# bbaaii/HFA-GP

Measured on AMD Instinct MI355X. Metric: rendered 512^2 frames/sec (96 depth samples), whole job, higher is better.
Workload: dtype f32 (conv GEMM products as f16x3: split 16-bit operands, fp32 accumulate); 1 GPU; ffhq512_128: synthesis fwd, 512^2 out, 128^2 rays x (48+48) samples, random-init weights (BASELINE config 2); parallelism=frame-parallel x1, conv_precision=f16x3

## Files before the change

hfa-gp_amd/_lib.py:

```python
from __future__ import annotations

import ctypes as C
import os
import threading

_HERE = os.path.dirname(os.path.abspath(__file__))
LIB_PATH = os.environ.get("HFAGP_LIB_PATH") or os.path.join(_HERE, "libhfagp_hip.so")
ABI_VERSION = 15

c_float_p = C.c_void_p


class RaymarchArgs(C.Structure):
    _fields_ = [
        ("planes", C.c_void_p), ("cam2world", C.c_void_p), ("intrinsics", C.c_void_p),
        ("u_strat", C.c_void_p), ("u_imp", C.c_void_p),
        ("dec_w0", C.c_void_p), ("dec_b0", C.c_void_p), ("dec_w1", C.c_void_p), ("dec_b1", C.c_void_p),
        ("feat", C.c_void_p), ("depth", C.c_void_p), ("wsum", C.c_void_p), ("tminmax", C.c_void_p),
        ("B", C.c_int32), ("H", C.c_int32), ("W", C.c_int32), ("res", C.c_int32),
        ("Sc", C.c_int32), ("Sf", C.c_int32), ("plane_axes", C.c_int32), ("white_back", C.c_int32),
        ("ray_start", C.c_double), ("ray_end", C.c_double),
        ("box_warp", C.c_float), ("decoder_lr_mul", C.c_float),
        ("planes_absmax", C.c_void_p), ("state", C.c_void_p),
    ]
# ... 90 lines not shown
class TorgbFinishArgs(C.Structure):
    _fields_ = [(n, C.c_void_p) for n in ("part", "bias", "rgb_in", "rgb_out", "y_pre")] + \
        [(n, C.c_int32) for n in ("nparts", "B", "H", "W", "Cout")] + [("clamp", C.c_float)]


class PointwiseBwdArgs(C.Structure):
    _fields_ = [(n, C.c_void_p) for n in (
        "dxs_conv", "s_conv", "dxs_rgb", "s_rgb", "g_rgb_small", "w_rgb_small", "s_small", "g_direct", "x",
        "dcoef_p", "bias_p", "noise_p", "g_out", "partial", "sums")] + \
        [(n, C.c_int32) for n in ("B", "H", "W", "C", "Co", "nchunks", "has_producer", "act_p", "param_grads")] + \
        [(n, C.c_float) for n in ("noise_strength_p", "alpha", "gain", "clamp")] + \
        [(n, C.c_void_p) for n in ("y_rgb_small", "g_nchw3_a", "g_nchw3_b")] + [("clamp_rgb_small", C.c_float)] + \
        [("noise_strength_dev", C.c_void_p)]


class StyleBwdArgs(C.Structure):
    _fields_ = [(n, C.c_void_p) for n in ("ds", "dd", "styles", "dcoef", "wsq", "affine_w", "dstot", "dw")] + \
        [(n, C.c_int32) for n in ("B", "Cin", "Cout", "w_dim", "dw_stride", "accumulate")] + \
        [("style_gain", C.c_float)]


class WgradArgs(C.Structure):
    _fields_ = [(n, C.c_void_p) for n in ("x", "styles", "g", "weight", "dd", "dcoef", "dweight", "workspace")] + \
        [(n, C.c_int32) for n in ("B", "H", "W", "Cin", "Cout", "mode", "ksplit", "precision", "accumulate", "dd_stride")]


class AffineGradItem(C.Structure):
    _fields_ = [(n, C.c_void_p) for n in ("dstot", "w", "dA", "db")] + [(n, C.c_int32) for n in ("B", "Cin", "w_dim", "w_stride")]


class ReducePartialsItem(C.Structure):
    _fields_ = [("partial", C.c_void_p), ("sums", C.c_void_p)] + [(n, C.c_int32) for n in ("B", "nchunks", "n")]


class BiasNoiseGradItem(C.Structure):
    _fields_ = [(n, C.c_void_p) for n in ("sums", "dbias", "dnoise")] + [(n, C.c_int32) for n in ("B", "C")]


class WeightPrepItem(C.Structure):
    _fields_ = [(n, C.c_void_p) for n in ("weight", "image", "image_t", "wsq")] + \
        [(n, C.c_int32) for n in ("Cout", "Cin", "taps", "precision", "precision_t")] + [("w_absmax", C.c_void_p)]


class StyleBwdItem(C.Structure):
    _fields_ = [(n, C.c_void_p) for n in ("ds", "dd", "styles", "dcoef", "wsq", "affine_w", "dstot", "dw")] + \
        [(n, C.c_int32) for n in ("B", "Cin", "Cout", "w_dim", "dw_stride", "ds_stride", "dd_stride")] + \
        [("style_gain", C.c_float)]


class RaymarchBwdArgs(C.Structure):
    _fields_ = [("fwd", RaymarchArgs), ("g_feat", C.c_void_p), ("d_planes", C.c_void_p), ("rec", C.c_void_p),
                ("d_dec_w0", C.c_void_p), ("d_dec_b0", C.c_void_p), ("d_dec_w1", C.c_void_p), ("d_dec_b1", C.c_void_p),
                ("df_scratch", C.c_void_p), ("rows_scratch", C.c_void_p), ("rows_scratch_bytes", C.c_uint64)]


class RaymarchGeomGrads(C.Structure):
    _fields_ = [("g_depth", C.c_void_p), ("g_wsum", C.c_void_p), ("depth_range", C.c_void_p)]


SYMBOLS = {
    "hfagp_abi_version": (C.c_int, []),
    "hfagp_last_error": (C.c_char_p, []),
    "hfagp_raymarch_fwd": (C.c_int, [C.POINTER(RaymarchArgs), C.c_void_p]),
    "hfagp_raymarch_normals": (C.c_int, [C.POINTER(RaymarchArgs), C.c_void_p, C.c_void_p]),
    "hfagp_raymarch_normals_bwd": (C.c_int, [C.POINTER(RaymarchArgs)] + [C.c_void_p] * 7),
    "hfagp_raymarch_normals_bwd_camera": (C.c_int, [C.POINTER(RaymarchArgs), C.c_void_p, C.c_void_p, C.c_int] + [C.c_void_p] * 3),
    "hfagp_planes_query": (C.c_int, [C.POINTER(PlanesQueryArgs), C.c_void_p]),
    "hfagp_planes_query_bwd": (C.c_int, [C.POINTER(PlanesQueryBwdArgs), C.c_void_p]),
    "hfagp_planes_query_normals": (C.c_int, [C.POINTER(PlanesQueryArgs), C.c_void_p, C.c_void_p, C.c_void_p]),
    "hfagp_planes_query_normals_bwd": (C.c_int, [C.POINTER(PlanesQueryBwdArgs), C.c_void_p, C.c_void_p, C.c_void_p]),
    "hfagp_marching_cubes_workspace_bytes": (C.c_size_t, [C.c_int32] * 3),
    "hfagp_marching_cubes_count": (C.c_int, [C.POINTER(MarchingCubesArgs), C.c_void_p]),
    "hfagp_marching_cubes_emit": (C.c_int, [C.POINTER(MarchingCubesArgs), C.c_void_p]),
    "hfagp_depth_clamp": (C.c_int, [C.c_void_p, C.c_void_p, C.c_int64, C.c_void_p]),
    "hfagp_style_fwd": (C.c_int, [C.POINTER(StyleArgs), C.c_void_p]),
    "hfagp_fc_fwd": (C.c_int, [C.c_void_p] * 4 + [C.c_int32] * 3 + [C.c_float, C.c_int32, C.c_float, C.c_float, C.c_void_p]),
    "hfagp_weight_prep": (C.c_int, [C.c_void_p, C.c_void_p, C.c_void_p, C.c_int32, C.c_int32, C.c_int32, C.c_void_p]),
    "hfagp_qr_gram_fwd": (C.c_int, [C.c_void_p, C.c_void_p, C.c_void_p, C.c_void_p, C.c_int32, C.c_void_p]),
    "hfagp_qr_refine_fwd": (C.c_int, [C.c_void_p, C.c_void_p, C.c_void_p, C.c_void_p, C.c_int32, C.c_void_p]),
    "hfagp_tall_gram_workspace_bytes": (C.c_size_t, [C.c_int32, C.c_int32]),
    "hfagp_tall_gram": (C.c_int, [C.c_void_p, C.c_int64, C.c_int64, C.c_void_p, C.c_int64, C.c_int64, C.c_void_p, C.c_void_p,
                                  C.c_int32, C.c_int32, C.c_float, C.c_void_p]),
    "hfagp_style_batch_fwd": (C.c_int, [C.POINTER(StyleArgs), C.c_int32, C.c_void_p]),
    "hfagp_weight_prep_split": (C.c_int, [C.c_void_p, C.c_void_p, C.c_int32, C.c_int32, C.c_int32, C.c_int32, C.c_void_p]),
    "hfagp_weight_prep_prec": (C.c_int, [C.c_void_p, C.c_void_p, C.c_int32, C.c_int32, C.c_int32, C.c_int32, C.c_void_p]),
    "hfagp_weight_prep_scaled": (C.c_int, [C.c_void_p, C.c_void_p, C.c_void_p, C.c_int32, C.c_int32, C.c_int32, C.c_int32, C.c_void_p]),
    "hfagp_modconv_workspace_bytes": (C.c_size_t, [C.POINTER(ModconvArgs)]),
    "hfagp_modconv_fwd": (C.c_int, [C.POINTER(ModconvArgs), C.c_void_p]),
    "hfagp_upfir_epilogue_fwd": (C.c_int, [C.POINTER(UpfirEpilogueArgs), C.c_void_p]),
    "hfagp_upconv_fir_scratch_bytes": (C.c_size_t, [C.POINTER(ModconvArgs)]),
    "hfagp_upconv_fir_fwd": (C.c_int, [C.POINTER(ModconvArgs), C.c_void_p, C.c_void_p]),
    "hfagp_skip_upsample_add": (C.c_int, [C.POINTER(SkipArgs), C.c_void_p]),
    "hfagp_torgb_skip_fwd": (C.c_int, [C.POINTER(TorgbSkipArgs), C.c_void_p]),
    "hfagp_blur_down_fwd": (C.c_int, [C.c_void_p, C.c_void_p, C.c_int32, C.c_int32, C.c_int32, C.c_int32, C.c_void_p]),
    "hfagp_blur_down_bwd": (C.c_int, [C.c_void_p, C.c_void_p, C.c_int32, C.c_int32, C.c_int32, C.c_int32, C.c_void_p]),
    "hfagp_torgb_fwd": (C.c_int, [C.POINTER(TorgbArgs), C.c_void_p]),
    "hfagp_torgb_finish_fwd": (C.c_int, [C.POINTER(TorgbFinishArgs), C.c_void_p]),
    "hfagp_modconv_rgb_parts": (C.c_int32, [C.POINTER(ModconvArgs)]),
    "hfagp_pointwise_bwd": (C.c_int, [C.POINTER(PointwiseBwdArgs), C.c_void_p]),
    "hfagp_upfir_bwd": (C.c_int, [C.c_void_p, C.c_void_p] + [C.c_int32] * 4 + [C.c_void_p]),
    "hfagp_upsample2d_bwd": (C.c_int, [C.c_void_p, C.c_void_p, C.c_int64, C.c_int32, C.c_int32, C.c_int32, C.c_void_p]),
    "hfagp_planes_to_nhwc": (C.c_int, [C.c_void_p, C.c_void_p] + [C.c_int32] * 4 + [C.c_void_p]),
    "hfagp_style_bwd": (C.c_int, [C.POINTER(StyleBwdArgs), C.c_void_p]),
    "hfagp_style_batch_bwd": (C.c_int, [C.POINTER(StyleBwdItem), C.c_int32, C.c_void_p]),
    "hfagp_raymarch_bwd": (C.c_int, [C.POINTER(RaymarchBwdArgs), C.c_void_p]),
    "hfagp_raymarch_bwd_geom": (C.c_int, [C.POINTER(RaymarchBwdArgs), C.POINTER(RaymarchGeomGrads), C.c_void_p]),
    "hfagp_raymarch_bwd_rows_bytes": (C.c_size_t, [C.POINTER(RaymarchArgs)]),
    "hfagp_raymarch_bwd_camera": (C.c_int, [C.POINTER(RaymarchBwdArgs), C.c_void_p, C.c_void_p, C.c_void_p, C.c_void_p]),
    "hfagp_adam_step": (C.c_int, [C.c_void_p, C.c_void_p, C.c_int32, C.c_int32, C.c_double, C.c_double, C.c_double, C.c_double, C.c_void_p]),
    "hfagp_adam_chunk": (C.c_int32, []),
    "hfagp_weight_prep_batch": (C.c_int, [C.POINTER(WeightPrepItem), C.c_int32, C.c_void_p]),
    "hfagp_wgrad_ksplit": (C.c_int32, [C.POINTER(WgradArgs)]),
    "hfagp_wgrad_workspace_bytes": (C.c_size_t, [C.POINTER(WgradArgs)]),
    "hfagp_conv_wgrad": (C.c_int, [C.POINTER(WgradArgs), C.c_void_p]),
    "hfagp_affine_grad": (C.c_int, [C.c_void_p] * 4 + [C.c_int32] * 4 + [C.c_void_p]),
    "hfagp_affine_grad_batch": (C.c_int, [C.POINTER(AffineGradItem), C.c_int32, C.c_void_p]),
    "hfagp_bias_noise_grads": (C.c_int, [C.POINTER(BiasNoiseGradItem), C.c_int32, C.c_void_p]),
    "hfagp_reduce_partials_batch": (C.c_int, [C.POINTER(ReducePartialsItem), C.c_int32, C.c_void_p]),
    "hfagp_channel_sum": (C.c_int, [C.c_void_p] * 3 + [C.c_int64, C.c_int32, C.c_int32, C.c_int32, C.c_void_p]),
    "hfagp_pool_mse_workspace_bytes": (C.c_size_t, []),
    "hfagp_pool_mse_fwd": (C.c_int, [C.c_void_p] * 5 + [C.c_int32] * 4 + [C.c_void_p]),
    "hfagp_pool_mse_bwd": (C.c_int, [C.c_void_p] * 4 + [C.c_int32] * 4 + [C.c_void_p]),
    "hfagp_upfirdn2d_fwd": (C.c_int, [C.c_void_p, C.c_void_p, C.c_void_p] + [C.c_int32] * 12 + [C.c_float, C.c_void_p]),
    "hfagp_upfirdn2d_bwd": (C.c_int, [C.c_void_p, C.c_void_p, C.c_void_p] + [C.c_int32] * 12 + [C.c_float, C.c_void_p]),
    "hfagp_bias_act_bwd": (C.c_int, [C.c_void_p, C.c_void_p, C.c_void_p, C.c_int64, C.c_int32, C.c_float, C.c_float,
                                     C.c_float, C.c_void_p]),
    "hfagp_bias_act_fwd": (C.c_int, [C.c_void_p, C.c_void_p, C.c_void_p, C.c_int64, C.c_int32, C.c_int64,
                                     C.c_int32, C.c_float, C.c_float, C.c_float, C.c_void_p]),
    "hfagp_allreduce_f32": (C.c_int, [C.c_void_p, C.c_size_t, C.c_void_p, C.c_int32, C.c_void_p]),
    "hfagp_nchw_to_nhwc": (C.c_int, [C.c_void_p, C.c_void_p] + [C.c_int32] * 4 + [C.c_void_p]),
    "hfagp_nhwc_to_nchw": (C.c_int, [C.c_void_p, C.c_void_p] + [C.c_int32] * 4 + [C.c_void_p]),
}

_lock = threading.Lock()
_lib = None


def lib() -> C.CDLL:
    global _lib
    if _lib is not None:
        return _lib
    with _lock:
        if _lib is not None:
            return _lib
        if not os.path.exists(LIB_PATH):
            raise RuntimeError(
                f"hfa_gp_amd: HIP library not found at {LIB_PATH}. There is no CPU fallback; build it with "
                f"`bash {os.path.join(_HERE, 'csrc', 'build.sh')}` (hipcc --offload-arch=gfx950).")
        try:
            import torch
            handle = C.CDLL(LIB_PATH)
        except OSError as e:
            raise RuntimeError(f"hfa_gp_amd: cannot load {LIB_PATH}: {e}") from e
        for name, (res, args) in SYMBOLS.items():
            try:
                fn = getattr(handle, name)
            except AttributeError as e:
                raise RuntimeError(f"hfa_gp_amd: {LIB_PATH} does not export {name}") from e
            fn.restype = res
            fn.argtypes = args
        ver = handle.hfagp_abi_version()
        if ver != ABI_VERSION:
            raise RuntimeError(f"hfa_gp_amd: ABI version mismatch: library {ver}, binding {ABI_VERSION}")
        _lib = handle
    return _lib

# ... 6 lines not shown
```

hfa-gp_amd/csrc/elementwise.hip:

```cpp
#include "common.h"

namespace hfagp {

static thread_local char g_err[512] = "";
void set_error(const char* fmt, ...) {
    va_list ap;
    va_start(ap, fmt);
    vsnprintf(g_err, sizeof(g_err), fmt, ap);
    va_end(ap);
}

__global__ void __launch_bounds__(256) style_kernel(const float* __restrict__ w, const float* __restrict__ A,
                                                    const float* __restrict__ ab, float* __restrict__ styles,
                                                    int B, int w_dim, int w_stride, int Cin, float wgain, float sgain) {
    const int wave = (blockIdx.x * blockDim.x + threadIdx.x) >> 6;
    const int lane = threadIdx.x & 63;
    if (wave >= B * Cin) return;
    const int b = wave / Cin, i = wave % Cin;
    const float* wr = w + (size_t)b * w_stride;
    const float* ar = A + (size_t)i * w_dim;
    float acc = 0.f;
    for (int k = lane * 4; k < w_dim; k += 256) {
        const float4 x = *reinterpret_cast<const float4*>(wr + k);
        const float4 y = *reinterpret_cast<const float4*>(ar + k);
        acc += x.x * y.x + x.y * y.y + x.z * y.z + x.w * y.w;
    }
    for (int o = 32; o > 0; o >>= 1) acc += __shfl_xor(acc, o);
    if (lane == 0) styles[wave] = (acc * wgain + ab[i]) * sgain;
}

__global__ void __launch_bounds__(256) demod_kernel(const float* __restrict__ styles, const float* __restrict__ wsq,
                                                    float* __restrict__ dcoef, int B, int Cin, int Cout, float eps) {
    const int wave = (blockIdx.x * blockDim.x + threadIdx.x) >> 6;
    const int lane = threadIdx.x & 63;
    if (wave >= B * Cout) return;
    const int b = wave / Cout, o = wave % Cout;
    const float* s = styles + (size_t)b * Cin;
    const float* q = wsq + (size_t)o * Cin;
    float acc = 0.f;
    for (int k = lane; k < Cin; k += 64) acc += s[k] * s[k] * q[k];
    for (int m = 32; m > 0; m >>= 1) acc += __shfl_xor(acc, m);
    if (lane == 0) dcoef[wave] = rsqrtf(acc + eps);
}

constexpr int kStyleBatch = 32;
struct StyleBatch { HfagpStyleArgs it[kStyleBatch]; };

__global__ void __launch_bounds__(256) style_batch_kernel(const StyleBatch t) {
    const HfagpStyleArgs& a = t.it[blockIdx.y];
    const int wave = (blockIdx.x * blockDim.x + threadIdx.x) >> 6;
    const int lane = threadIdx.x & 63;
    if (wave >= a.B * a.Cin) return;
    const int b = wave / a.Cin, i = wave % a.Cin;
    const float* wr = a.w + (size_t)b * a.w_stride;
    const float* ar = a.affine_w + (size_t)i * a.w_dim;
    float acc = 0.f;
    for (int k = lane * 4; k < a.w_dim; k += 256) {
        const float4 x = *reinterpret_cast<const float4*>(wr + k);
        const float4 y = *reinterpret_cast<const float4*>(ar + k);
        acc += x.x * y.x + x.y * y.y + x.z * y.z + x.w * y.w;
    }
    for (int o = 32; o > 0; o >>= 1) acc += __shfl_xor(acc, o);
    if (lane == 0) a.styles[wave] = (acc * rsqrtf((float)a.w_dim) + a.affine_b[i]) * a.style_gain;
}

__global__ void __launch_bounds__(256) demod_batch_kernel(const StyleBatch t) {
    const HfagpStyleArgs& a = t.it[blockIdx.y];
    if (!a.dcoef) return;
    const int wave = (blockIdx.x * blockDim.x + threadIdx.x) >> 6;
    const int lane = threadIdx.x & 63;
    if (wave >= a.B * a.Cout) return;
    const int b = wave / a.Cout, o = wave % a.Cout;
    const float* s = a.styles + (size_t)b * a.Cin;
    const float* q = a.wsq + (size_t)o * a.Cin;
    float acc = 0.f;
    for (int k = lane; k < a.Cin; k += 64) acc += s[k] * s[k] * q[k];
    for (int m = 32; m > 0; m >>= 1) acc += __shfl_xor(acc, m);
    if (lane == 0) a.dcoef[wave] = rsqrtf(acc + a.eps);
}

__global__ void __launch_bounds__(256) fc_kernel(const float* __restrict__ x, const float* __restrict__ W,
                                                 const float* __restrict__ bias, float* __restrict__ y, int B, int In,
                                                 int Out, float wgain, float bgain, int act, float alpha, float gain) {
    const int wave = (blockIdx.x * blockDim.x + threadIdx.x) >> 6, lane = threadIdx.x & 63;
    if (wave >= B * Out) return;
    const int b = wave / Out, o = wave % Out;
    float acc = 0.f;
    for (int k = lane; k < In; k += 64) acc += x[(size_t)b * In + k] * W[(size_t)o * In + k];
    for (int m = 32; m > 0; m >>= 1) acc += __shfl_xor(acc, m);
    if (lane == 0) y[wave] = lrelu_gain_clamp(acc * wgain + (bias ? bias[o] * bgain : 0.f), act, alpha, gain, -1.f);
}

__global__ void __launch_bounds__(256) weight_prep_kernel(const float* __restrict__ w, float* __restrict__ wt,
                                                          float* __restrict__ wsq, int Cout, int Cin, int taps) {
    const int idx = blockIdx.x * blockDim.x + threadIdx.x;
    if (idx >= Cout * Cin) return;
    const int co = idx / Cin, ci = idx % Cin;
    const float* src = w + (size_t)idx * taps;
    float sq = 0.f;
    for (int t = 0; t < taps; ++t) {
        const float v = src[t];
        sq += v * v;
        wt[(((size_t)t * (Cin >> 2) + (ci >> 2)) * Cout + co) * 4 + (ci & 3)] = v;
    }
    if (wsq) wsq[idx] = sq;
}

#ifndef HFAGP_FIR_STRIP
#define HFAGP_FIR_STRIP 8
#endif
constexpr int kStrip = HFAGP_FIR_STRIP;

typedef _Float16 h2_t __attribute__((ext_vector_type(2)));
typedef float f2_t __attribute__((ext_vector_type(2)));
template <bool H16>
__device__ __forceinline__ float4 load4(const void* base, size_t idx4) {
    if constexpr (H16) {
        const uint2 u = reinterpret_cast<const uint2*>(base)[idx4];
        const h2_t a = __builtin_bit_cast(h2_t, u.x), b = __builtin_bit_cast(h2_t, u.y);
        return make_float4((float)a[0], (float)a[1], (float)b[0], (float)b[1]);
    } else {
        return reinterpret_cast<const float4*>(base)[idx4];
    }
}
template <bool H16>
__device__ __forceinline__ void store4(void* base, size_t idx4, float4 v) {
    if constexpr (H16) {
        const f2_t lo = {v.x, v.y}, hi = {v.z, v.w};
        reinterpret_cast<uint2*>(base)[idx4] = make_uint2(__builtin_bit_cast(unsigned, __builtin_convertvector(lo, h2_t)),
                                                          __builtin_bit_cast(unsigned, __builtin_convertvector(hi, h2_t)));
    } else {
        reinterpret_cast<float4*>(base)[idx4] = v;
    }
}

template <bool H16>
__global__ void __launch_bounds__(256) upfir_epilogue_kernel(HfagpUpfirEpilogueArgs a) {
    const int C4 = a.C >> 2;
    const int Wo = 2 * a.W, Ho = 2 * a.H, Wi = 2 * a.W + 1, Hi = 2 * a.H + 1;
    const int Wp = a.W;
    const int strips = (Ho + kStrip - 1) / kStrip;
    const long long total = (long long)a.B * strips * Wp * C4;
    const long long tid = (long long)blockIdx.x * blockDim.x + threadIdx.x;
    if (tid >= total) return;
    const int c4 = (int)(tid % C4);
    const int X = 2 * (int)((tid / C4) % Wp);
    const int st = (int)((tid / ((long long)C4 * Wp)) % strips);
    const int b = (int)(tid / ((long long)C4 * Wp * strips));
    const int Y0 = st * kStrip;
    const size_t src0 = (size_t)b * Hi * Wi * C4 + c4;
    const float f0 = 0.25f, f1 = 0.75f;

    int xo[5]; float xm[5];
#pragma unroll
// ... 313 lines not shown
    for (int p = 0; p < fh; ++p) {
        const int uy = oy * down + p - py0;
        if (uy < 0 || uy % up != 0) continue;
        const int iy = uy / up;
        if (iy >= H) continue;
        for (int q = 0; q < fw; ++q) {
            const int ux = ox * down + q - px0;
            if (ux < 0 || ux % up != 0) continue;
            const int ix = ux / up;
            if (ix >= W) continue;
            acc += (noflip ? f[p * fw + q] : f[(fh - 1 - p) * fw + (fw - 1 - q)]) * src[(size_t)iy * W + ix];
        }
    }
    y[tid] = acc * gain;
}

__global__ void __launch_bounds__(256) bias_act_kernel(const float* __restrict__ x, const float* __restrict__ b,
                                                       float* __restrict__ y, long long n, int C, long long inner,
                                                       int act, float alpha, float gain, float clamp) {
    const long long stride = (long long)gridDim.x * blockDim.x;
    for (long long i = (long long)blockIdx.x * blockDim.x + threadIdx.x; i < n; i += stride) {
        float v = x[i];
        if (b) v += b[(i / inner) % C];
        y[i] = lrelu_gain_clamp(v, act, alpha, gain, clamp);
    }
}

__global__ void __launch_bounds__(256) bias_act_bwd_kernel(const float* __restrict__ dy, const float* __restrict__ y,
                                                           float* __restrict__ dx, long long n, int act, float alpha,
                                                           float gain, float clamp) {
    const long long stride = (long long)gridDim.x * blockDim.x;
    for (long long i = (long long)blockIdx.x * blockDim.x + threadIdx.x; i < n; i += stride) {
        const float yv = y[i];
        float g = dy[i] * gain;
        if (act == HFAGP_ACT_LRELU && !(yv > 0.f)) g *= alpha;
        if (clamp >= 0.f && !(fabsf(yv) < clamp)) g = 0.f;
        dx[i] = g;
    }
}

__global__ void __launch_bounds__(256) transpose_kernel(const float* __restrict__ x, float* __restrict__ y,
                                                        int rows, int cols) {
    __shared__ float tile[32][33];
    const size_t base = (size_t)blockIdx.z * rows * cols;
    const int c0 = blockIdx.x * 32, r0 = blockIdx.y * 32;
    const int tx = threadIdx.x & 31, ty = threadIdx.x >> 5;
    for (int k = ty; k < 32; k += 8) {
        const int r = r0 + k, c = c0 + tx;
        if (r < rows && c < cols) tile[k][tx] = x[base + (size_t)r * cols + c];
    }
    __syncthreads();
    for (int k = ty; k < 32; k += 8) {
        const int c = c0 + k, r = r0 + tx;
        if (r < rows && c < cols) y[base + (size_t)c * rows + r] = tile[tx][k];
    }
}

}

using namespace hfagp;

extern "C" {

int hfagp_abi_version(void) { return HFAGP_ABI_VERSION; }
const char* hfagp_last_error(void) { return g_err; }

int hfagp_style_fwd(const HfagpStyleArgs* a, void* stream) {
    HFAGP_REQUIRE(a && a->w && a->affine_w && a->affine_b && a->styles, HFAGP_EBADARG, "style_fwd: null pointer");
    HFAGP_REQUIRE(a->B > 0 && a->Cin > 0 && a->w_dim > 0 && a->w_dim % 4 == 0 && a->w_stride % 4 == 0,
                  HFAGP_EBADARG, "style_fwd: bad dims B=%d Cin=%d w_dim=%d", a->B, a->Cin, a->w_dim);
    hipStream_t s = (hipStream_t)stream;
    const float wgain = 1.0f / sqrtf((float)a->w_dim);
    int waves = a->B * a->Cin;
    style_kernel<<<(waves + 3) / 4, 256, 0, s>>>(a->w, a->affine_w, a->affine_b, a->styles, a->B, a->w_dim,
                                                 a->w_stride, a->Cin, wgain, a->style_gain);
    if (a->dcoef) {
        HFAGP_REQUIRE(a->wsq && a->Cout > 0, HFAGP_EBADARG, "style_fwd: dcoef requested without wsq");
        waves = a->B * a->Cout;
        demod_kernel<<<(waves + 3) / 4, 256, 0, s>>>(a->styles, a->wsq, a->dcoef, a->B, a->Cin, a->Cout, a->eps);
    }
    return check_launch("style_fwd");
}

int hfagp_style_batch_fwd(const HfagpStyleArgs* items, int32_t n, void* stream) {
    HFAGP_REQUIRE(items && n >= 1 && n <= kStyleBatch, HFAGP_EBADARG, "style_batch_fwd: 1..%d items, got %d", kStyleBatch, n);
    StyleBatch t;
    int max_s = 0, max_d = 0;
    for (int i = 0; i < n; ++i) {
        const HfagpStyleArgs& a = items[i];
        HFAGP_REQUIRE(a.w && a.affine_w && a.affine_b && a.styles, HFAGP_EBADARG, "style_batch_fwd: null pointer in item %d", i);
        HFAGP_REQUIRE(a.B > 0 && a.Cin > 0 && a.w_dim > 0 && a.w_dim % 4 == 0 && a.w_stride % 4 == 0, HFAGP_EBADARG,
                      "style_batch_fwd: bad dims in item %d: B=%d Cin=%d w_dim=%d", i, a.B, a.Cin, a.w_dim);
        HFAGP_REQUIRE(!a.dcoef || (a.wsq && a.Cout > 0), HFAGP_EBADARG, "style_batch_fwd: item %d: dcoef without wsq", i);
        t.it[i] = a;
        max_s = a.B * a.Cin > max_s ? a.B * a.Cin : max_s;
        if (a.dcoef) max_d = a.B * a.Cout > max_d ? a.B * a.Cout : max_d;
    }
    hipStream_t s = (hipStream_t)stream;
    style_batch_kernel<<<dim3((max_s + 3) / 4, n), 256, 0, s>>>(t);
    if (max_d) demod_batch_kernel<<<dim3((max_d + 3) / 4, n), 256, 0, s>>>(t);
    return check_launch("style_batch_fwd");
}

int hfagp_fc_fwd(const float* x, const float* weight, const float* bias, float* y, int32_t B, int32_t In, int32_t Out,
                 float lr_mul, int32_t act, float alpha, float gain, void* stream) {
    HFAGP_REQUIRE(x && weight && y, HFAGP_EBADARG, "fc_fwd: null pointer");
    HFAGP_REQUIRE(B > 0 && In > 0 && Out > 0, HFAGP_EBADARG, "fc_fwd: bad dims");
    HFAGP_REQUIRE(act == HFAGP_ACT_LINEAR || act == HFAGP_ACT_LRELU, HFAGP_EUNSUPPORTED, "fc_fwd: act %d", act);
    const int waves = B * Out;
    fc_kernel<<<(waves + 3) / 4, 256, 0, (hipStream_t)stream>>>(x, weight, bias, y, B, In, Out,
                                                                lr_mul / sqrtf((float)In), lr_mul, act, alpha, gain);
    return check_launch("fc_fwd");
}

int hfagp_weight_prep(const float* weight, float* wt, float* wsq, int32_t Cout, int32_t Cin, int32_t taps,
                      void* stream) {
    HFAGP_REQUIRE(weight && wt, HFAGP_EBADARG, "weight_prep: null pointer");
    HFAGP_REQUIRE(Cin % 4 == 0 && Cout > 0 && (taps == 1 || taps == 9), HFAGP_EUNSUPPORTED,
                  "weight_prep: Cin=%d must be a multiple of 4, taps=%d must be 1 or 9", Cin, taps);
    const int n = Cout * Cin;
    weight_prep_kernel<<<(n + 255) / 256, 256, 0, (hipStream_t)stream>>>(weight, wt, wsq, Cout, Cin, taps);
    return check_launch("weight_prep");
}

int hfagp_upfir_epilogue_fwd(const HfagpUpfirEpilogueArgs* a, void* stream) {
    HFAGP_REQUIRE(a && a->yt && a->y, HFAGP_EBADARG, "upfir_epilogue: null pointer");
    HFAGP_REQUIRE(a->C % 4 == 0 && a->B > 0 && a->H > 0 && a->W > 0, HFAGP_EUNSUPPORTED,
                  "upfir_epilogue: C=%d must be a multiple of 4", a->C);
    const int strips = (2 * a->H + kStrip - 1) / kStrip;
    const long long total = (long long)a->B * strips * a->W * (a->C / 4);
    if (a->io_f16) upfir_epilogue_kernel<true><<<(unsigned)((total + 255) / 256), 256, 0, (hipStream_t)stream>>>(*a);
    else upfir_epilogue_kernel<false><<<(unsigned)((total + 255) / 256), 256, 0, (hipStream_t)stream>>>(*a);
    return check_launch("upfir_epilogue");
}

int hfagp_skip_upsample_add(const HfagpSkipArgs* a, void* stream) {
    HFAGP_REQUIRE(a && a->y && a->img_out, HFAGP_EBADARG, "skip_upsample_add: null pointer");
    HFAGP_REQUIRE(a->C % 4 == 0 && (!a->plane_major || (a->C % 3 == 0 && (a->C / 3) % 4 == 0)), HFAGP_EUNSUPPORTED,
                  "skip_upsample_add: unsupported channel count %d", a->C);
    const int Ho = a->img_in ? 2 * a->H : a->H, Wo = a->img_in ? 2 * a->W : a->W;
    const long long total = (long long)a->B * Ho * Wo * (a->C / 4);
    skip_kernel<<<(unsigned)((total + 255) / 256), 256, 0, (hipStream_t)stream>>>(*a);
    return check_launch("skip_upsample_add");
}

int hfagp_torgb_fwd(const HfagpTorgbArgs* a, void* stream) {
    HFAGP_REQUIRE(a && a->x && a->weight && a->styles && a->bias && a->rgb_out, HFAGP_EBADARG, "torgb: null pointer");
    HFAGP_REQUIRE(a->Cout >= 1 && a->Cout <= kTorgbMaxOut && a->Cin % 4 == 0 && a->H % 2 == 0 && a->W % 2 == 0,
                  HFAGP_EUNSUPPORTED, "torgb: Cout=%d (max %d), Cin=%d", a->Cout, kTorgbMaxOut, a->Cin);
    const int HW = a->H * a->W;
    hipStream_t s = (hipStream_t)stream;
    const dim3 rgrid((HW + 32 * kTorgbIter - 1) / (32 * kTorgbIter), a->B);
    switch (a->Cin) {
        case 64:  if (a->Cout <= 3) torgb_reg_kernel<2, 3><<<rgrid, 256, 0, s>>>(*a); else torgb_reg_kernel<2, 4><<<rgrid, 256, 0, s>>>(*a); break;
        case 128: if (a->Cout <= 3) torgb_reg_kernel<4, 3><<<rgrid, 256, 0, s>>>(*a); else torgb_reg_kernel<4, 4><<<rgrid, 256, 0, s>>>(*a); break;
        case 256: if (a->Cout <= 3) torgb_reg_kernel<8, 3><<<rgrid, 256, 0, s>>>(*a); else torgb_reg_kernel<8, 4><<<rgrid, 256, 0, s>>>(*a); break;
        default: {
            dim3 grid((HW + 31) / 32, a->B);
            const size_t lds = (size_t)a->Cout * a->Cin * sizeof(float);
            torgb_kernel<<<grid, 256, lds, s>>>(*a);
        }
    }
    return check_launch("torgb");
}

int hfagp_torgb_finish_fwd(const HfagpTorgbFinishArgs* a, void* stream) {
    HFAGP_REQUIRE(a && a->part && a->bias && a->rgb_out, HFAGP_EBADARG, "torgb_finish: null pointer");
    HFAGP_REQUIRE(a->Cout >= 1 && a->Cout <= 3 && a->nparts >= 1 && a->H % 2 == 0 && a->W % 2 == 0, HFAGP_EUNSUPPORTED,
                  "torgb_finish: Cout=%d (max 3), nparts=%d", a->Cout, a->nparts);
    const long long total = (long long)a->B * a->H * a->W;
    torgb_finish_kernel<<<(unsigned)((total + 255) / 256), 256, 0, (hipStream_t)stream>>>(*a);
    return check_launch("torgb_finish");
}

int hfagp_blur_down_fwd(const float* x, float* y, int32_t B, int32_t H, int32_t W, int32_t C, void* stream) {
    HFAGP_REQUIRE(x && y, HFAGP_EBADARG, "blur_down: null pointer");
    HFAGP_REQUIRE(B > 0 && H > 0 && W > 0 && H % 2 == 0 && W % 2 == 0 && C % 4 == 0, HFAGP_EUNSUPPORTED,
                  "blur_down: H=%d, W=%d must be even and C=%d a multiple of 4", H, W, C);
    const long long total = (long long)B * (H / 2) * (W / 2) * (C / 4);
    blur_down_kernel<<<(unsigned)((total + 255) / 256), 256, 0, (hipStream_t)stream>>>(x, y, B, H, W, C / 4);
    return check_launch("blur_down_fwd");
}

int hfagp_blur_down_bwd(const float* gy, float* gx, int32_t B, int32_t H, int32_t W, int32_t C, void* stream) {
// ... 72 lines not shown
```

hfa-gp_amd/csrc/modconv.hip:

```cpp
#include "modconv_plan.h"

namespace hfagp {

typedef float f32x16 __attribute__((ext_vector_type(16)));

constexpr int CK = 8;
constexpr int AS = 12;
constexpr int LPW = 32;

template <int WM, int WN, int TM, int TN>
__global__ void __launch_bounds__(256) modconv_kernel(const ConvParams p) {
    constexpr int BM = WM * TM * 32, BN = WN * TN * 32, PH = BM / PW;
    extern __shared__ __attribute__((aligned(16))) float lds[];
    float* As = lds;
    float* Bs = lds + ((PH + 2) * LPW) * AS;

    const Phase& ph = p.phase[blockIdx.y];
    unsigned id = blockIdx.x;
    const int tn_blk = __builtin_amdgcn_readfirstlane(id % p.tiles_n); id /= p.tiles_n;
    const int tw = __builtin_amdgcn_readfirstlane(id % p.tiles_w);     id /= p.tiles_w;
    const int th = __builtin_amdgcn_readfirstlane(id % p.tiles_h);     id /= p.tiles_h;
    const int b = __builtin_amdgcn_readfirstlane(id % p.B);            id /= p.B;
    const int ks = __builtin_amdgcn_readfirstlane(id);
    const int m0 = th * PH, n0 = tw * PW, co0 = tn_blk * BN;
    if (m0 >= ph.mh || n0 >= ph.mw) return;

    const int tid = threadIdx.x, lane = tid & 63, wave = tid >> 6;
    const int wm = wave / WN, wn = wave % WN;
    const int h = lane >> 5, l31 = lane & 31;

    const int c_begin = __builtin_amdgcn_readfirstlane((int)(((long long)p.nchunks * ks) / p.ksplit));
    const int c_end = __builtin_amdgcn_readfirstlane((int)(((long long)p.nchunks * (ks + 1)) / p.ksplit));

    const int npatch = p.ph * p.pw;
    constexpr int A_PER_T = ((PH + 2) * (PW + 2) * 2 + 255) / 256;
    constexpr int B_PER_T = (MAXTAPS * 2 * BN + 255) / 256;
    float4 ra[A_PER_T], rs[A_PER_T], rb[B_PER_T];
    const float* xb = p.x + ph.in_off + (long long)b * p.x_batch_stride;
    const float* sb = p.styles ? p.styles + (size_t)b * p.Cin : nullptr;
    const int nB = ph.ntaps * 2 * BN;
    const int cq = p.Cin >> 2;

    long long aoff[A_PER_T], boff[B_PER_T];
    int lds_a[A_PER_T];
#pragma unroll
    for (int k = 0; k < A_PER_T; ++k) {
        const int idx = tid + k * 256;
        aoff[k] = -1;
        lds_a[k] = 0;
        if (idx < npatch * 2) {
            const int pix = idx >> 1, q = idx & 1;
            lds_a[k] = ((pix / p.pw) * LPW + pix % p.pw) * AS + 4 * q;
            const int iy = m0 + p.dymin + pix / p.pw, ix = n0 + p.dxmin + pix % p.pw;
            if (iy >= 0 && iy < p.in_h && ix >= 0 && ix < p.in_w) aoff[k] = ((long long)iy * p.in_w + ix) * p.Cin + 4 * q;
        }
    }
#pragma unroll
    for (int k = 0; k < B_PER_T; ++k) {
        const int idx = tid + k * 256;
        boff[k] = -1;
        if (idx < nB) {
            const int co = idx % BN, q = (idx / BN) & 1, t = idx / (2 * BN);
            if (co0 + co < p.Cout) boff[k] = ((long long)ph.widx[t] * cq + q) * p.Cout + co0 + co;
        }
    }

    auto load_regs = [&](int chunk) {
        const int c0 = chunk * CK;
#pragma unroll
        for (int k = 0; k < A_PER_T; ++k) {
            float4 v = make_float4(0.f, 0.f, 0.f, 0.f), sv = make_float4(1.f, 1.f, 1.f, 1.f);
            if (aoff[k] >= 0) {
                v = *reinterpret_cast<const float4*>(xb + aoff[k] + c0);
                if (sb) sv = *reinterpret_cast<const float4*>(sb + c0 + 4 * ((tid + k * 256) & 1));
            }
            ra[k] = v; rs[k] = sv;
        }
#pragma unroll
        for (int k = 0; k < B_PER_T; ++k) {
            float4 v = make_float4(0.f, 0.f, 0.f, 0.f);
            if (boff[k] >= 0) v = reinterpret_cast<const float4*>(p.wt)[boff[k] + (long long)(c0 >> 2) * p.Cout];
            rb[k] = v;
        }
// ... 90 lines not shown
                const int m = m0 + (pidx >> 4), n = n0 + (pidx & 15);
                if (m >= ph.mh || n >= ph.mw) continue;
                const int oy = ph.sy * m + ph.oy0, ox = ph.sx * n + ph.ox0;
                float v = acc[tm][tn][r];
                if (p.fused) {
                    v = v * d + bs + nz[r] * p.noise_strength;
                    v = lrelu_gain_clamp(v, p.act, p.alpha, p.gain, p.clamp);
                }
                vmax = fmaxf(vmax, fabsf(v));
                out[(((size_t)b * p.Ho + oy) * p.Wo + ox) * p.Cout + co] = v;
            }
        }
    }
    if (p.fused && p.y_absmax) publish_absmax(p.y_absmax, vmax, blockIdx.x * 4 + (threadIdx.x >> 6));
}

__global__ void __launch_bounds__(256) splitk_epilogue_kernel(const float* __restrict__ ws, float* __restrict__ y,
                                                              const float* __restrict__ dcoef,
                                                              const float* __restrict__ noise,
                                                              const float* __restrict__ bias, long long slab,
                                                              int ksplit, int HoWo, int Cout, int fused, int act,
                                                              float noise_strength, float alpha, float gain,
                                                              float clamp, float* __restrict__ y_absmax) {
    const long long i4 = (long long)blockIdx.x * blockDim.x + threadIdx.x;
    if (i4 * 4 >= slab) return;
    float4 s = reinterpret_cast<const float4*>(ws)[i4];
    int k = 1;
    for (; k + 8 <= ksplit; k += 8) {
        float4 v[8];
#pragma unroll
        for (int q = 0; q < 8; ++q) v[q] = reinterpret_cast<const float4*>(ws + (size_t)(k + q) * slab)[i4];
#pragma unroll
        for (int q = 0; q < 8; ++q) { s.x += v[q].x; s.y += v[q].y; s.z += v[q].z; s.w += v[q].w; }
    }
    for (; k < ksplit; ++k) {
        const float4 v = reinterpret_cast<const float4*>(ws + (size_t)k * slab)[i4];
        s.x += v.x; s.y += v.y; s.z += v.z; s.w += v.w;
    }
    if (fused) {
        const long long e = i4 * 4;
        const int co = (int)(e % Cout);
        const long long pix = e / Cout;
        const int b = (int)(pix / HoWo);
        float4 d = make_float4(1.f, 1.f, 1.f, 1.f), bs = make_float4(0.f, 0.f, 0.f, 0.f);
        if (dcoef) d = *reinterpret_cast<const float4*>(dcoef + (size_t)b * Cout + co);
        if (bias) bs = *reinterpret_cast<const float4*>(bias + co);
        const float nz = noise ? noise[pix % HoWo] * noise_strength : 0.f;
        s.x = lrelu_gain_clamp(s.x * d.x + bs.x + nz, act, alpha, gain, clamp);
        s.y = lrelu_gain_clamp(s.y * d.y + bs.y + nz, act, alpha, gain, clamp);
        s.z = lrelu_gain_clamp(s.z * d.z + bs.z + nz, act, alpha, gain, clamp);
        s.w = lrelu_gain_clamp(s.w * d.w + bs.w + nz, act, alpha, gain, clamp);
    }
    reinterpret_cast<float4*>(y)[i4] = s;
    if (fused && y_absmax)
        publish_absmax(y_absmax, fmaxf(fmaxf(fabsf(s.x), fabsf(s.y)), fmaxf(fabsf(s.z), fabsf(s.w))), blockIdx.x * 4 + (threadIdx.x >> 6));
}

}

using namespace hfagp;

extern "C" {

static int resolve_modconv(const HfagpModconvArgs* a, Plan& pl) {
    const int ck = a && a->precision != HFAGP_PREC_F32 ? 16 : CK;
    int rc = validate(a, ck);
    if (rc == HFAGP_OK) rc = make_plan(a, pl, ck);
    if (rc != HFAGP_OK) return rc;
    pl.small = smallconv_takes(a);
    if (pl.small) {
        pl.p.ksplit = smallconv_ksplit(a);
        pl.ws_bytes = pl.p.ksplit > 1 ? (size_t)pl.p.ksplit * pl.p.slab * sizeof(float) : 0;
    }
    return HFAGP_OK;
}

size_t hfagp_modconv_workspace_bytes(const HfagpModconvArgs* a) {
    Plan pl;
    return resolve_modconv(a, pl) == HFAGP_OK ? pl.ws_bytes : 0;
}

int32_t hfagp_modconv_rgb_parts(const HfagpModconvArgs* a) { return a ? ((a->Cout + 127) / 128) * 2 : 0; }

int hfagp_modconv_fwd(const HfagpModconvArgs* a, void* stream) {
    Plan pl;
    int rc = resolve_modconv(a, pl);
    if (rc != HFAGP_OK) return rc;
    ConvParams& p = pl.p;
    HFAGP_REQUIRE((a->rgb_w == nullptr) == (a->rgb_part == nullptr), HFAGP_EBADARG, "modconv: rgb_w and rgb_part go together");
    if (pl.small) {
        rc = launch_smallconv(a, pl, (hipStream_t)stream);
        if (rc != HFAGP_OK || p.ksplit == 1) return rc;
        const long long n4 = p.slab / 4;
        splitk_epilogue_kernel<<<(unsigned)((n4 + 255) / 256), 256, 0, (hipStream_t)stream>>>(
            a->workspace, a->y, a->dcoef, a->noise, a->bias, p.slab, p.ksplit, p.Ho * p.Wo, a->Cout, 1, a->act,
            a->noise_strength, a->alpha, a->gain, a->clamp, a->y_absmax);
        return check_launch("modconv_fwd/splitk (small-image kernel)");
    }
    HFAGP_REQUIRE(!a->rgb_part || (a->precision != HFAGP_PREC_F32 && p.ksplit * p.nslab == 1 && p.fused && a->Cout % 128 == 0 &&
                                   (a->mode == HFAGP_CONV3X3 || a->mode == HFAGP_CONV1X1)),
                  HFAGP_EUNSUPPORTED, "modconv: the fused toRGB needs a 16-bit precision, mode 0 / 2, Cout %% 128 == 0 and no "
                                      "split-K (workspace_bytes() == 0); got precision %d mode %d Cout %d ksplit %d",
                  a->precision, a->mode, a->Cout, p.ksplit);
    HFAGP_REQUIRE(a->y || (a->rgb_part && !a->y_absmax), HFAGP_EBADARG,
                  "modconv: y may only be NULL with the fused toRGB (rgb_w / rgb_part) and without y_absmax");
    hipStream_t s = (hipStream_t)stream;
    const int nslabs = p.ksplit * p.nslab;
    if (nslabs > 1) {
        HFAGP_REQUIRE(a->workspace, HFAGP_EBADARG, "modconv: split-K (%d slabs) needs a workspace of %zu bytes", nslabs,
                      pl.ws_bytes);
        p.out = a->workspace;
    } else {
        p.out = a->y;
    }
    HFAGP_REQUIRE(!(a->x_f16 || a->y_f16) || a->precision == HFAGP_PREC_F16, HFAGP_EUNSUPPORTED,
                  "modconv: fp16 storage (x_f16 / y_f16) goes with precision HFAGP_PREC_F16");
    if (a->precision != HFAGP_PREC_F32) {
        rc = launch_modconv_bf16(a, pl, s);
        if (rc != HFAGP_OK) return rc;
    } else {
        const size_t lds_bytes = ((size_t)(pl.bm / PW + 2) * LPW * AS + (size_t)MAXTAPS * 2 * pl.bn * 4) * sizeof(float);
        switch (pl.bn) {
            case 128: modconv_kernel<2, 2, 2, 2><<<pl.grid, 256, lds_bytes, s>>>(p); break;
            case 96:  modconv_kernel<4, 1, 1, 3><<<pl.grid, 256, lds_bytes, s>>>(p); break;
            case 64:  modconv_kernel<2, 2, 2, 1><<<pl.grid, 256, lds_bytes, s>>>(p); break;
            default:  modconv_kernel<4, 1, 1, 1><<<pl.grid, 256, lds_bytes, s>>>(p); break;
        }
        rc = check_launch("modconv_fwd");
        if (rc != HFAGP_OK) return rc;
    }
    if (nslabs > 1) {
        const int fused = a->mode != HFAGP_CONVT3X3_UP2 && a->mode != HFAGP_CONVS2_BWD;
        const long long n4 = p.slab / 4;
        splitk_epilogue_kernel<<<(unsigned)((n4 + 255) / 256), 256, 0, s>>>(
            a->workspace, a->y, a->dcoef, a->noise, a->bias, p.slab, nslabs, p.Ho * p.Wo, a->Cout, fused, a->act,
            a->noise_strength, a->alpha, a->gain, a->clamp, a->y_absmax);
        rc = check_launch("modconv_fwd/splitk");
    }
    return rc;
}

}
```

hfa-gp_amd/csrc/modconv_bf16.hip:

```cpp
#include <atomic>
#include <type_traits>
#include "conv16_common.h"

namespace hfagp {

template <int KD, int TM, int NTAPS, int IO = 0>
__global__ void __launch_bounds__(256, 2) modconv_bf16_kernel(const ConvParams p, const int phase0) {
    constexpr int NP = kind_parts_a(KD), NPB = kind_parts(KD);
    constexpr bool F16 = kind_f16(KD);
    constexpr bool XH = (IO & 1) != 0, YH = (IO & 2) != 0;
    constexpr int XB = XH ? 2 : 4;
    static_assert((IO & 3) == 0 || KD == 1, "fp16 storage goes with the single-pass fp16 arithmetic");
    constexpr bool ELEG = (IO & 4) != 0;
    static_assert(!ELEG || (KD == 4 && NTAPS == 9 && IO == 4), "the legacy epilogue is kept for one instantiation");
    constexpr int WN = 2, WM = 4 / WN, TN = 4 / WN, TMW = 4 / WM, BM = 128, PH = BM / PW;
    static_assert(TM == 2, "block tile is 128 positions");
    constexpr int LPWB = RowPitch<NP>::value;
    constexpr int APOS = (PH + 2) * LPWB;
    constexpr int A_PART = APOS * APITCH, A_BUF = NP * A_PART;
    extern __shared__ __attribute__((aligned(16))) char lds_raw[];
    char* As = lds_raw;
    float* Ss = reinterpret_cast<float*>(lds_raw + 2 * A_BUF);

    constexpr bool MERGED_S2 = NTAPS == 0;
// ... 342 lines not shown
            for (int rw = 0; rw < 2; ++rw) {
                const int m = m0 + 2 * (wm * TMW + tm) + rw;
                if (m >= ph.mh) continue;
                const int oy = ph.sy * m + ph.oy0;
                const size_t rowoff = (((size_t)b * p.Ho + oy) * p.Wo + ph.ox0) * p.Cout + co;
                float* rowp = out + rowoff;
                _Float16* rowh = reinterpret_cast<_Float16*>(p.out) + rowoff;
                const float* nrow = (p.fused && p.noise) ? p.noise + (size_t)oy * p.Wo + ph.ox0 : nullptr;
                float nz[8];
#pragma unroll
                for (int q = 0; q < 8; ++q) {
                    const int n = min(n0 + 8 * (q >> 2) + 4 * h + (q & 3), ph.mw - 1);
                    nz[q] = nrow ? nrow[ph.sx * n] * p.noise_strength : 0.f;
                }
#pragma unroll
                for (int q = 0; q < 8; ++q) {
                    const int n = n0 + 8 * (q >> 2) + 4 * h + (q & 3);
                    if (n >= ph.mw) continue;
                    float v = acc[tm][tn][8 * rw + q];
                    if (p.fused) v = lrelu_gain_clamp(v * d + bs + nz[q], p.act, p.alpha, p.gain, p.clamp);
                    else if constexpr (F16) v *= sback;
                    vmax = fmaxf(vmax, fabsf(v));
                    if (p.out) {
                        if constexpr (YH) rowh[n * cstep] = (_Float16)v;
                        else rowp[n * cstep] = v;
                    }
                    if constexpr (RGB) {
#pragma unroll
                        for (int r = 0; r < 3; ++r)
                            rgbp[((tm * 2 + rw) * 8 + q) * 3 + r] = fmaf(v, rw3[r], rgbp[((tm * 2 + rw) * 8 + q) * 3 + r]);
                    }
                }
            }
    }
    if (p.fused && p.y_absmax) publish_absmax(p.y_absmax, vmax, blockIdx.x * 4 + wave);
    }
    if constexpr (RGB) {
        if (do_rgb) {
            int n = TMW * 16 * 3;
#pragma unroll
            for (int m = 16; m >= 1; m >>= 1) {
                n >>= 1;
                const bool up = (l31 & m) != 0;
#pragma unroll
                for (int i = 0; i < TMW * 16 * 3 / 2; ++i) {
                    if (i < n) {
                        const float keep = up ? rgbp[i + n] : rgbp[i];
                        const float give = up ? rgbp[i] : rgbp[i + n];
                        rgbp[i] = keep + __shfl_xor(give, m);
                    }
                }
            }
            const int pos = l31;
            const int tm = pos >> 4, rw = (pos >> 3) & 1, q = pos & 7;
            const int m = m0 + 2 * (wm * TMW + tm) + rw, nn = n0 + 8 * (q >> 2) + 4 * h + (q & 3);
            if (m < ph.mh && nn < ph.mw) {
                const int part = tn_blk * WN + wn;
                float4* dst = reinterpret_cast<float4*>(p.rgb_part) +
                              (((size_t)part * p.B + b) * p.Ho + (ph.sy * m + ph.oy0)) * p.Wo + (ph.sx * nn + ph.ox0);
                *dst = make_float4(rgbp[0], rgbp[1], rgbp[2], 0.f);
            }
        }
    }
}

constexpr int UP4_OCC = 2;
template <int KD, int NW, int IO = 0>
__global__ void __launch_bounds__(NW * 64, (NW == 4 && KD != 3) ? UP4_OCC : 1) upconv_bf16_kernel(const ConvParams p) {
    constexpr int NP = kind_parts_a(KD), NPB = kind_parts(KD);
    constexpr bool F16 = kind_f16(KD);
    constexpr bool XH = (IO & 1) != 0, YH = (IO & 2) != 0;
    constexpr int XB = XH ? 2 : 4;
    static_assert(IO == 0 || KD == 1, "fp16 storage goes with the single-pass fp16 arithmetic");
    constexpr int NTH = NW * 64;
    constexpr int TM = 2, TN = 1, WN = NW / 2, BM = 128, BNU = WN * TN * 32, PH = BM / PW, RB = kind_nprod(KD) == 1 ? 6 : 3;
    constexpr int LPWB = RowPitch<NP>::value;
    constexpr int APOS = (PH + 2) * LPWB;
    constexpr int A_PART = APOS * APITCH, A_BUF = NP * A_PART;
    using namespace up_items;
    extern __shared__ __attribute__((aligned(16))) char lds_raw[];
    char* As = lds_raw;
    float* Ss = reinterpret_cast<float*>(lds_raw + 2 * A_BUF);

    unsigned id = p.xcd ? xcd_remap(blockIdx.x, gridDim.x) : blockIdx.x;
    const int tiles_nu = p.Cout / BNU;
    const int tn_blk = __builtin_amdgcn_readfirstlane(id % tiles_nu);  id /= tiles_nu;
    const int n_reg = p.up_tr * p.up_tw, n_tile = n_reg + p.up_nf;
    const int T = __builtin_amdgcn_readfirstlane(id % n_tile);         id /= n_tile;
    const int ks = __builtin_amdgcn_readfirstlane(id);
    const bool fringe = T >= n_reg;
    const int RP = p.up_rp, R_total = p.up_rows;
    const int r0 = fringe ? (T - n_reg) * 64 : (T / p.up_tw) * PH, n0 = fringe ? 0 : (T % p.up_tw) * PW;
    const int co0 = tn_blk * BNU;
    const int b_lo = min(max(r0 - 1, 0) / RP, p.B - 1);

    const int tid = threadIdx.x, lane = tid & 63, wave = tid >> 6;
    const int wm = wave / WN, wn = wave % WN;
    const int h = lane >> 5, l31 = lane & 31;
    const int c_begin = __builtin_amdgcn_readfirstlane((int)(((long long)p.nchunks * ks) / p.ksplit));
    const int c_end = __builtin_amdgcn_readfirstlane((int)(((long long)p.nchunks * (ks + 1)) / p.ksplit));

    const int npatch = p.ph * p.pw;
    constexpr int A_PER_T = ((PH + 2) * (PW + 2) * 4 + NTH - 1) / NTH;
    static_assert(A_PER_T == 2 || A_PER_T == 3, "staging schedule: two or three slots per thread");
    float4 ra[A_PER_T];
    const char* xb = reinterpret_cast<const char*>(p.x) + (long long)b_lo * p.x_batch_stride * XB;
    float* Gd = Ss + p.up_ns * p.Cin;
    {
        const long long s_lo = (long long)b_lo * p.Cin, s_n = (long long)p.B * p.Cin;
        for (int i = tid; i < p.up_ns * p.Cin; i += NTH) Ss[i] = (p.styles && s_lo + i < s_n) ? p.styles[s_lo + i] : 1.f;
        for (int sI = 0; sI < p.up_ns; ++sI) {
            float bk = 1.f, dn = 1.f;
            if constexpr (F16)
                dn = style_range_guard((p.styles && b_lo + sI < p.B) ? p.styles + (size_t)(b_lo + sI) * p.Cin : nullptr, p.Cin, lane, &bk,
                                       p.x_absmax, p.w_absmax);
            if (tid == 0) { Gd[sI] = dn; Gd[p.up_ns + sI] = bk; }
        }
    }
    __syncthreads();
    unsigned aoff[A_PER_T];
    int lds_a[A_PER_T], soff[A_PER_T];
    float amask[A_PER_T];
#pragma unroll
    for (int k = 0; k < A_PER_T; ++k) {
        const int idx = min(tid + k * NTH, npatch * 4 - 1);
        const int pix = idx >> 2, q = idx & 3;
        const int pi = pix / p.pw, pj = pix % p.pw;
        lds_a[k] = (pi * LPWB + pj) * APITCH + 8 * q;
        int r, n;
        if (!fringe) { r = r0 - 1 + pi; n = n0 - 1 + pj; }
        else { r = pj == 0 ? -1 : r0 + 8 * ((pj - 1) >> 1) + pi - 1; n = p.W - 1 + ((pj - 1) & 1); }
        const bool row_ok = r >= 0 && r < R_total;
        const int bb = row_ok ? r / RP : b_lo, m = r - bb * RP;
        const bool inside = row_ok && m < p.H && n >= 0 && n < p.W;
        const int sel = inside ? bb - b_lo : 0;
        aoff[k] = inside ? (unsigned)(((long long)sel * p.x_batch_stride + (long long)(m * p.W + n) * p.Cin + 4 * q) * XB) : 0u;
        amask[k] = inside ? Gd[sel] : 0.f;
        soff[k] = sel * p.Cin + 4 * q;
    }
    auto load_a = [&](int chunk) __attribute__((always_inline)) { a16_load<XH>(ra, xb, chunk, aoff); };
    auto store_a = [&](int chunk, auto buf_tag, auto k_tag) __attribute__((always_inline)) {
        constexpr int BUF = decltype(buf_tag)::value, k = decltype(k_tag)::value;
        a16_store<KD, XH>(As + BUF * A_BUF, A_PART, lds_a[k], amask[k], *reinterpret_cast<const float4*>(Ss + chunk * CKB + soff[k]), ra[k]);
    };

    const char* wb = reinterpret_cast<const char*>(p.wt);
    const int cq8 = p.Cin >> 3;
    const int part_stride = 9 * cq8 * p.Cout;
    unsigned bth[TN];
#pragma unroll
    for (int tn = 0; tn < TN; ++tn) bth[tn] = (unsigned)(h * p.Cout + co0 + (wn * TN + tn) * 32 + l31) * 16u;
    int apos[TM];
#pragma unroll
    for (int tm = 0; tm < TM; ++tm) {
        const int pidx = (wm * TM + tm) * 32 + l31;
        apos[tm] = ((pidx >> 4) * LPWB + (pidx & 15)) * APITCH + 16 * h;
    }

    f32x16 acc[4][TM][TN];
#pragma unroll
    for (int f = 0; f < 4; ++f)
#pragma unroll
        for (int tm = 0; tm < TM; ++tm)
#pragma unroll
            for (int tn = 0; tn < TN; ++tn)
#pragma unroll
                for (int r = 0; r < 16; ++r) acc[f][tm][tn][r] = 0.f;

    constexpr PartOrder PO = kind_order(KD);
    constexpr int NPROD = PO.nprod;
    u32x4 bq[RB][TN][NPB];
    u32x4 af[2][TM][NP];
    auto issue_b = [&](int c, auto i_tag, auto slot_tag) __attribute__((always_inline)) {
        constexpr int I = decltype(i_tag)::value, SL = decltype(slot_tag)::value;
        const int cc = min(c, c_end - 1);
#pragma unroll
        for (int q = 0; q < NPB; ++q) {
            const char* base = wb + (long long)(q * part_stride + (I_W[I] * cq8 + cc * 2) * p.Cout) * 16;
#pragma unroll
            for (int tn = 0; tn < TN; ++tn) bq[SL][tn][q] = *reinterpret_cast<const u32x4*>(base + bth[tn]);
        }
    };
    auto read_a = [&](auto u_tag, auto g_tag) __attribute__((always_inline)) {
        constexpr int UU = decltype(u_tag)::value, G = decltype(g_tag)::value;
#pragma unroll
        for (int tm = 0; tm < TM; ++tm)
#pragma unroll
            for (int q = 0; q < NP; ++q)
                af[G & 1][tm][q] = *reinterpret_cast<const u32x4*>(As + UU * A_BUF + q * A_PART + group_pos(G, LPWB) * APITCH + apos[tm]);
    };
    auto item = [&](int c, auto u_tag, auto i_tag) __attribute__((always_inline)) {
        constexpr int I = decltype(i_tag)::value, G = I_GRP[I], F = I_PHASE[I];
        constexpr int SL = (decltype(u_tag)::value * NITEM + I) % RB;
        if constexpr (I == G_FIRST[G] && G < 3) read_a(u_tag, std::integral_constant<int, G + 1>{});
        __builtin_amdgcn_sched_barrier(0);
#pragma unroll
        for (int pr = 0; pr < NPROD; ++pr)
#pragma unroll
            for (int tm = 0; tm < TM; ++tm)
// ... 366 lines not shown
    for (int tn = 0; tn < 4; ++tn) {
        const int co = co0 + wn * 64 + tn * 16 + i16;
        float rw3[3] = {0.f, 0.f, 0.f};
        if (do_rgb) {
#pragma unroll
            for (int r = 0; r < 3; ++r) rw3[r] = p.rgb_w[((size_t)b * 3 + r) * p.Cout + co];
        }
        float d = sback, bs = 0.f;
        if (p.fused) {
            if (p.dcoef) d = p.dcoef[(size_t)b * p.Cout + co] * sback;
            if (p.bias) bs = p.bias[co];
        }
#pragma unroll
        for (int tm = 0; tm < 4; ++tm) {
            const int m = m0 + 4 * wm + tm;
            if (m >= p.Ho) continue;
            float* rowp = out + ((size_t)b * p.Ho + m) * p.Wo * p.Cout + co;
            const float* nrow = (p.fused && p.noise) ? p.noise + (size_t)m * p.Wo : nullptr;
#pragma unroll
            for (int r = 0; r < 4; ++r) {
                const int n = n0 + 4 * g + r;
                const float nz = nrow ? nrow[min(n, p.Wo - 1)] * p.noise_strength : 0.f;
                if (n >= p.Wo) continue;
                float v = acc[tm][tn][r];
                if (p.fused) v = lrelu_gain_clamp(v * d + bs + nz, p.act, p.alpha, p.gain, p.clamp);
                else v *= sback;
                vmax = fmaxf(vmax, fabsf(v));
                if (p.out) rowp[n * p.Cout] = v;
#pragma unroll
                for (int c = 0; c < 3; ++c) rgbp[(tm * 4 + r) * 3 + c] = fmaf(v, rw3[c], rgbp[(tm * 4 + r) * 3 + c]);
            }
        }
    }
    if (p.fused && p.y_absmax) publish_absmax(p.y_absmax, vmax, blockIdx.x * 4 + wave);
    }
    if (do_rgb) {
        int n = 16 * 3;
#pragma unroll
        for (int mk = 8; mk >= 1; mk >>= 1) {
            n >>= 1;
            const bool up = (i16 & mk) != 0;
#pragma unroll
            for (int i = 0; i < 16 * 3 / 2; ++i) {
                if (i < n) {
                    const float keep = up ? rgbp[i + n] : rgbp[i];
                    const float give = up ? rgbp[i] : rgbp[i + n];
                    rgbp[i] = keep + __shfl_xor(give, mk);
                }
            }
        }
        const int m = m0 + 4 * wm + (i16 >> 2), nn = n0 + 4 * g + (i16 & 3);
        if (m < p.Ho && nn < p.Wo) {
            const int part = tn_blk * 2 + wn;
            float4* dst = reinterpret_cast<float4*>(p.rgb_part) + (((size_t)part * p.B + b) * p.Ho + m) * p.Wo + nn;
            *dst = make_float4(rgbp[0], rgbp[1], rgbp[2], 0.f);
        }
    }
}

namespace u16 {
constexpr int CK = 32;
constexpr int LP = PW + 1, NPOS = (8 + 1) * LP;
constexpr int OCT = 2560;
constexpr int A_PART = 4 * OCT, A_BUF = 2 * A_PART;
constexpr int A_PER_T = 5;
constexpr unsigned OOB = 0xfffff000u;
static_assert(NPOS * 16 <= OCT && OCT % 256 == 0 && NPOS * 8 <= A_PER_T * 256 && 2 * A_BUF <= 48 * 1024, "patch layout");
constexpr size_t lds_bytes(int cin, int ns) { return (size_t)2 * A_BUF + (size_t)ns * (cin + 1) * sizeof(float); }
}

template <int KD, int NW, int IO, int LOOP>
__global__ void __launch_bounds__(256, 2) upconv_bf16_kernel(const ConvParams p) {
    static_assert(KD == 4 && NW == 4 && IO == 0 && LOOP == 2, "the 32-channel loop is the 4-wave F16X3 up-conv");
    using namespace u16;
    typedef float f32x4v __attribute__((ext_vector_type(4)));
    using namespace up_items;
    constexpr int RB = 2;
    constexpr int ST = 0;
    constexpr int S_SLOT[NITEM] = {-1, -1, 0, 1, -1, 2, 3, -1, 4};
    extern __shared__ __attribute__((aligned(16))) char lds_raw[];
    char* As = lds_raw;
    float* Ss = reinterpret_cast<float*>(lds_raw + 2 * A_BUF);

    unsigned id = p.xcd ? xcd_remap(blockIdx.x, gridDim.x) : blockIdx.x;
    const int tiles_nu = p.Cout / 64;
    const int tn_blk = __builtin_amdgcn_readfirstlane(id % tiles_nu);  id /= tiles_nu;
    const int n_reg = p.up_tr * p.up_tw, n_tile = n_reg + p.up_nf;
    const int T = __builtin_amdgcn_readfirstlane(id % n_tile);         id /= n_tile;
    const int ks = __builtin_amdgcn_readfirstlane(id);
    const bool fringe = T >= n_reg;
    const int RP = p.up_rp, R_total = p.up_rows;
    const int r0 = fringe ? (T - n_reg) * 64 : (T / p.up_tw) * 8, n0 = fringe ? 0 : (T % p.up_tw) * PW;
    const int co0 = tn_blk * 64;
    const int b_lo = min(max(r0 - 1, 0) / RP, p.B - 1);

    const int tid = threadIdx.x, lane = tid & 63, wave = __builtin_amdgcn_readfirstlane(tid >> 6);
    const int wm = wave >> 1, wn = wave & 1;
    const int g = lane >> 4, i16 = lane & 15;
    const int nch = p.Cin / CK;
    const int c_begin = __builtin_amdgcn_readfirstlane((int)(((long long)nch * ks) / p.ksplit));
    const int c_end = __builtin_amdgcn_readfirstlane((int)(((long long)nch * (ks + 1)) / p.ksplit));

    float* Gb = Ss + p.up_ns * p.Cin;
    for (int sI = 0; sI < p.up_ns; ++sI) {
        const float* st = (p.styles && b_lo + sI < p.B) ? p.styles + (size_t)(b_lo + sI) * p.Cin : nullptr;
        float bk = 1.f;
        const float dn = style_range_guard(st, p.Cin, lane, &bk, p.x_absmax, p.w_absmax);
        for (int i = tid; i < p.Cin; i += 256) Ss[sI * p.Cin + i] = (st ? st[i] : 1.f) * dn;
        if (tid == 0) Gb[sI] = bk;
    }

    const int nsamp = min(p.up_ns, p.B - b_lo);
    const __amdgpu_buffer_rsrc_t rx = __builtin_amdgcn_make_buffer_rsrc(
        const_cast<float*>(p.x + (long long)b_lo * p.x_batch_stride), 0,
        (unsigned)(((long long)(nsamp - 1) * p.x_batch_stride + (long long)p.H * p.W * p.Cin) * 4), 0x00020000);
    const int qa = 2 * ((tid >> 4) & 3) + (tid & 1);
    static_assert(A_PART <= (1 << 14) && 14 + 3 * A_PER_T <= 32, "LDS address and sample indices share a register");
    unsigned aoff[A_PER_T];
    unsigned sels = (qa >> 1) * OCT + (8 * (tid >> 6) + ((tid >> 1) & 7)) * 16 + (qa & 1) * 8;
#pragma unroll
    for (int k = 0; k < A_PER_T; ++k) {
        const int pix = 8 * ((tid >> 6) + 4 * k) + ((tid >> 1) & 7);
        const int pi = pix / LP, pj = pix % LP;
        int r, n;
        if (!fringe) { r = r0 - 1 + pi; n = n0 - 1 + pj; }
        else { r = pj == 0 ? -1 : r0 + 8 * ((pj - 1) >> 1) + pi - 1; n = p.W - 1 + ((pj - 1) & 1); }
        const bool row_ok = r >= 0 && r < R_total;
        const int bb = row_ok ? r / RP : b_lo, m = r - bb * RP;
        const bool inside = pix < NPOS && row_ok && m < p.H && n >= 0 && n < p.W;
        const int sel = inside ? bb - b_lo : 0;
        aoff[k] = inside ? (unsigned)(((long long)sel * p.x_batch_stride + (long long)(m * p.W + n) * p.Cin + 4 * qa) * 4) : OOB;
        sels |= (unsigned)sel << (14 + 3 * k);
    }
    static_assert((8 * (3 + 4 * (A_PER_T - 1)) + 7) * 16 < OCT, "every slot lies inside its octet");
    float4 ra[2];
    auto load_a = [&](int chunk, auto part_tag) __attribute__((always_inline)) {
        constexpr int PT = decltype(part_tag)::value;
#pragma unroll
        for (int k = 0; k < (PT < 2 ? 2 : 1); ++k)
            ra[k] = __builtin_bit_cast(float4, __builtin_amdgcn_raw_buffer_load_b128(rx, aoff[PT * 2 + k], chunk * CK * 4, 0));
    };
    auto store_a = [&](int chunk, auto buf_tag, auto k_tag) __attribute__((always_inline)) {
        constexpr int BUF = decltype(buf_tag)::value, k = decltype(k_tag)::value;
        const int sel = (int)((sels >> (14 + 3 * k)) & 7u);
        const float4 sv = *reinterpret_cast<const float4*>(Ss + chunk * CK + sel * p.Cin + 4 * qa);
        const int lds_a = (int)(sels & 0x3fffu) + k * 32 * 16;
        const float4 x = ra[k % 2];
        uint2 parts[2];
        split4<KD>(make_float4(x.x * sv.x, x.y * sv.y, x.z * sv.z, x.w * sv.w), parts);
#pragma unroll
        for (int q = 0; q < 2; ++q) *reinterpret_cast<uint2*>(As + BUF * A_BUF + q * A_PART + lds_a) = parts[q];
    };

    const int cq8 = p.Cin >> 3;
    const __amdgpu_buffer_rsrc_t rw = __builtin_amdgcn_make_buffer_rsrc(
        const_cast<void*>(p.wt), 0, (unsigned)(2 * 9 * cq8 * p.Cout) * 16u, 0x00020000);
    const unsigned boff = (unsigned)(g * p.Cout + co0 + wn * 32 + i16) * 16u;
    const int part_bytes = 9 * cq8 * p.Cout * 16, tap_bytes = cq8 * p.Cout * 16, chunk_bytes = 4 * p.Cout * 16;
    const char* const afrag = As + g * OCT + (4 * wm * LP + i16) * 16;

    f32x4v acc[4][4][2];
#pragma unroll
    for (int f = 0; f < 4; ++f)
#pragma unroll
        for (int tm = 0; tm < 4; ++tm)
#pragma unroll
            for (int tn = 0; tn < 2; ++tn) acc[f][tm][tn] = f32x4v{0.f, 0.f, 0.f, 0.f};

    constexpr PartOrder PO = kind_order(KD);
    u32x4 bq[RB][2][2];
    u32x4 af[4][2];
    auto issue_b = [&](int c, int w, auto slot_tag) __attribute__((always_inline)) {
        constexpr int SL = decltype(slot_tag)::value;
#pragma unroll
        for (int q = 0; q < 2; ++q) {
            const int so = q * part_bytes + w * tap_bytes + c * chunk_bytes;
#pragma unroll
            for (int tn = 0; tn < 2; ++tn) bq[SL][tn][q] = __builtin_amdgcn_raw_buffer_load_b128(rw, boff + 256 * tn, so, 0);
        }
    };
    auto read_a = [&](auto u_tag, auto g_tag, auto tm_tag) __attribute__((always_inline)) {
        constexpr int UU = decltype(u_tag)::value, G = decltype(g_tag)::value, TMI = decltype(tm_tag)::value;
#pragma unroll
        for (int q = 0; q < 2; ++q)
            af[TMI][q] = *reinterpret_cast<const u32x4*>(afrag + UU * A_BUF + q * A_PART + (TMI * LP + group_pos(G, LP)) * 16);
    };
    auto item = [&](int c, auto u_tag, auto i_tag) __attribute__((always_inline)) {
        constexpr int UU = decltype(u_tag)::value, I = decltype(i_tag)::value, G = I_GRP[I], F = I_PHASE[I];
        constexpr int SL = (UU * NITEM + I) % RB, IN = I + RB - 1;
        issue_b(c + IN / NITEM, I_W[IN % NITEM], std::integral_constant<int, (SL + RB - 1) % RB>{});
        if constexpr (I == 0) load_a(min(c + 1, c_end - 1), std::integral_constant<int, 0>{});
        __builtin_amdgcn_sched_barrier(0);
        auto tile = [&](auto tm_tag) __attribute__((always_inline)) {
            constexpr int TMI = decltype(tm_tag)::value;
#pragma unroll
            for (int pr = 0; pr < 3; ++pr)
#pragma unroll
                for (int tn = 0; tn < 2; ++tn) {
                    const f16x8 xa = __builtin_bit_cast(f16x8, af[TMI][PO.pa[pr]]), wb = __builtin_bit_cast(f16x8, bq[SL][tn][PO.pb[pr]]);
                    acc[F][TMI][tn] = __builtin_amdgcn_mfma_f32_16x16x32_f16(wb, xa, acc[F][TMI][tn], 0, 0, 0);
                }
            if constexpr (I + 1 < NITEM && I_GRP[(I + 1) % NITEM] != G) read_a(u_tag, std::integral_constant<int, G + 1>{}, tm_tag);
            if constexpr (TMI == ST && S_SLOT[I] >= 0)
                store_a(min(c + 1, c_end - 1), std::integral_constant<int, 1 - UU>{}, std::integral_constant<int, (S_SLOT[I] < 0 ? 0 : S_SLOT[I])>{});
            if constexpr (TMI == ST && (I == 3 || I == 6))
                load_a(min(c + 1, c_end - 1), std::integral_constant<int, I / 3>{});
            __builtin_amdgcn_sched_barrier(0);
        };
        tile(std::integral_constant<int, 0>{});
        tile(std::integral_constant<int, 1>{});
        tile(std::integral_constant<int, 2>{});
        tile(std::integral_constant<int, 3>{});
    };
    auto chunk = [&](int c, auto u_tag) __attribute__((always_inline)) {
        __syncthreads();
        read_a(u_tag, std::integral_constant<int, 0>{}, std::integral_constant<int, 0>{});
        read_a(u_tag, std::integral_constant<int, 0>{}, std::integral_constant<int, 1>{});
// ... 230 lines not shown
```

hfa-gp_amd/csrc/modconv_plan.h:

```cpp
#pragma once
#include <algorithm>
#include <cstdlib>
#include "common.h"

namespace hfagp {

constexpr int PW = 16;
constexpr int MAXTAPS = 9;

struct Phase {
    int ntaps;
    int mh, mw;
    int sy, sx, oy0, ox0;
    int slab;
    long long in_off;
    signed char dy[MAXTAPS], dx[MAXTAPS], widx[MAXTAPS];
};

struct ConvParams {
    const float* x; const void* wt; const float* styles; const float* dcoef;
    const float* noise; const float* bias;
    const float* x_absmax; float* y_absmax;
    const float* w_absmax;
    const float* rgb_w; float* rgb_part;
    int x_f16, y_f16;
    float* out;
    long long x_batch_stride;
    long long slab;
    int B, H, W, Cin, Cout, Ho, Wo;
    int in_h, in_w;
    int nphase, nslab, tiles_h, tiles_w, tiles_n, ksplit, nchunks;
    int wtaps;
    int dymin, dxmin, ph, pw;
    int fused;
    int up_rp, up_rows, up_tr, up_tw, up_nf, up_ns;
    int xcd;
    int act; float noise_strength, alpha, gain, clamp;
    Phase phase[4];
};

struct Plan {
    ConvParams p;
    int bn;
    int bm;
    dim3 grid;
    bool merged_up;
    bool merged_s2;
    bool small;
    int up_waves;
    size_t ws_bytes;
};

static inline void set_phase(Phase& ph, int ntaps, int mh, int mw, int sy, int sx, int oy0, int ox0,
                      const int (*taps)[3], int slab = 0, long long in_off = 0) {
    ph.ntaps = ntaps; ph.mh = mh; ph.mw = mw; ph.sy = sy; ph.sx = sx; ph.oy0 = oy0; ph.ox0 = ox0;
    ph.slab = slab; ph.in_off = in_off;
    for (int t = 0; t < ntaps; ++t) {
        ph.dy[t] = (signed char)taps[t][0]; ph.dx[t] = (signed char)taps[t][1]; ph.widx[t] = (signed char)taps[t][2];
    }
}

static inline int make_plan(const HfagpModconvArgs* a, Plan& pl, int ck) {
    ConvParams& p = pl.p;
    p = ConvParams{};
    p.x = a->x; p.wt = a->wt; p.styles = a->styles; p.dcoef = a->dcoef; p.noise = a->noise; p.bias = a->bias;
    p.x_absmax = a->x_absmax; p.y_absmax = a->y_absmax; p.w_absmax = a->w_absmax;
    p.rgb_w = a->rgb_w; p.rgb_part = a->rgb_part;
    p.x_f16 = a->x_f16; p.y_f16 = a->y_f16;
    p.x_batch_stride = a->x_batch_stride;
    p.B = a->B; p.H = a->H; p.W = a->W; p.Cin = a->Cin; p.Cout = a->Cout;
    p.act = a->act; p.noise_strength = a->noise_strength; p.alpha = a->alpha; p.gain = a->gain; p.clamp = a->clamp;
    p.nchunks = a->Cin / ck;
    { static const char* dev = getenv("HFAGP_DEV_XCD_REMAP"); p.xcd = dev ? atoi(dev) : 0; }
    p.nslab = 1;
    int in_h = a->H, in_w = a->W;

    if (a->Cout % 128 == 0 || a->precision != HFAGP_PREC_F32) pl.bn = 128;
    else if (a->Cout % 96 == 0) pl.bn = 96;
    else if (a->Cout % 64 == 0) pl.bn = 64;
    else pl.bn = 32;
    pl.bm = 128;
    const int PH = pl.bm / PW;
    p.tiles_n = (a->Cout + pl.bn - 1) / pl.bn;

    int gh, gw;
    if (a->mode == HFAGP_CONV3X3) {
        static const int t9[9][3] = {{-1, -1, 0}, {-1, 0, 1}, {-1, 1, 2}, {0, -1, 3}, {0, 0, 4},
                                     {0, 1, 5},   {1, -1, 6}, {1, 0, 7},  {1, 1, 8}};
        p.nphase = 1; p.Ho = a->H; p.Wo = a->W;
        set_phase(p.phase[0], 9, a->H, a->W, 1, 1, 0, 0, t9);
        p.dymin = -1; p.dxmin = -1; p.ph = PH + 2; p.pw = PW + 2;
        gh = a->H; gw = a->W; p.fused = 1;
    } else if (a->mode == HFAGP_CONV1X1) {
        static const int t1[1][3] = {{0, 0, 0}};
        p.nphase = 1; p.Ho = a->H; p.Wo = a->W;
        set_phase(p.phase[0], 1, a->H, a->W, 1, 1, 0, 0, t1);
        p.dymin = 0; p.dxmin = 0; p.ph = PH; p.pw = PW;
        gh = a->H; gw = a->W; p.fused = 1;
    } else if (a->mode == HFAGP_CONVT3X3_UP2) {
        static const int t00[4][3] = {{0, 0, 0}, {-1, 0, 6}, {0, -1, 2}, {-1, -1, 8}};
        static const int t01[2][3] = {{0, 0, 1}, {-1, 0, 7}};
        static const int t10[2][3] = {{0, 0, 3}, {0, -1, 5}};
        static const int t11[1][3] = {{0, 0, 4}};
        p.nphase = 4; p.Ho = 2 * a->H + 1; p.Wo = 2 * a->W + 1;
        set_phase(p.phase[0], 4, a->H + 1, a->W + 1, 2, 2, 0, 0, t00);
        set_phase(p.phase[1], 2, a->H + 1, a->W, 2, 2, 0, 1, t01);
        set_phase(p.phase[2], 2, a->H, a->W + 1, 2, 2, 1, 0, t10);
        set_phase(p.phase[3], 1, a->H, a->W, 2, 2, 1, 1, t11);
        p.dymin = -1; p.dxmin = -1; p.ph = PH + 1; p.pw = PW + 1;
        gh = a->H + 1; gw = a->W + 1; p.fused = 0;
    } else if (a->mode == HFAGP_CONV3X3_BWD) {
        static const int t9[9][3] = {{-1, -1, 8}, {-1, 0, 7}, {-1, 1, 6}, {0, -1, 5}, {0, 0, 4},
                                     {0, 1, 3},   {1, -1, 2}, {1, 0, 1},  {1, 1, 0}};
        p.nphase = 1; p.Ho = a->H; p.Wo = a->W;
        set_phase(p.phase[0], 9, a->H, a->W, 1, 1, 0, 0, t9);
        p.dymin = -1; p.dxmin = -1; p.ph = PH + 2; p.pw = PW + 2;
        gh = a->H; gw = a->W; p.fused = 1;
    } else if (a->mode == HFAGP_CONVS2_BWD) {
        static const int t00[4][3] = {{0, 0, 0}, {1, 0, 6}, {0, 1, 2}, {1, 1, 8}};
        static const int t01[2][3] = {{0, 0, 1}, {1, 0, 7}};
        static const int t10[2][3] = {{0, 0, 3}, {0, 1, 5}};
// ... 110 lines not shown
```

hfa-gp_amd/csrc/split_mfma.h:

```cpp
#pragma once
#include "common.h"

namespace hfagp {

typedef float f32x16 __attribute__((ext_vector_type(16)));
typedef __bf16 bf16x8 __attribute__((ext_vector_type(8)));
typedef __bf16 bf16x2 __attribute__((ext_vector_type(2)));
typedef float f32x2 __attribute__((ext_vector_type(2)));
typedef unsigned u32x4 __attribute__((ext_vector_type(4)));
typedef _Float16 f16x8 __attribute__((ext_vector_type(8)));
typedef _Float16 f16x2 __attribute__((ext_vector_type(2)));

constexpr int CKB = 16;
__device__ __forceinline__ unsigned pack_bf16(float a, float b) {
    const f32x2 v = {a, b};
    return __builtin_bit_cast(unsigned, __builtin_convertvector(v, bf16x2));
}

__device__ __forceinline__ unsigned pack_f16(float a, float b) {
    const f32x2 v = {a, b};
    return __builtin_bit_cast(unsigned, __builtin_convertvector(v, f16x2));
}

constexpr int kind_parts(int kd) { return kd == 4 || kd == 5 ? 2 : kd; }
constexpr int kind_parts_a(int kd) { return kd == 5 ? 1 : kind_parts(kd); }
constexpr int kind_split(int kd) { return kd == 5 ? 1 : kd; }
constexpr bool kind_f16(int kd) { return kd == 1 || kd == 4 || kd == 5; }
constexpr int kind_nprod(int kd) { return kd == 1 ? 1 : kd == 5 ? 2 : kind_parts(kd) == 2 ? 3 : 6; }
constexpr int kind_pa(int kd, int i) { return kd == 5 ? 0 : (i == 1 || i == 3) ? 1 : i == 4 ? 2 : 0; }
constexpr int kind_pb(int kd, int i) { return kd == 5 ? i : (i == 2 || i == 3) ? 1 : i == 5 ? 2 : 0; }
struct PartOrder { int nprod, pa[6], pb[6]; };
constexpr PartOrder kind_order(int kd) {
    return PartOrder{kind_nprod(kd), {kind_pa(kd, 0), kind_pa(kd, 1), kind_pa(kd, 2), kind_pa(kd, 3), kind_pa(kd, 4), kind_pa(kd, 5)},
                     {kind_pb(kd, 0), kind_pb(kd, 1), kind_pb(kd, 2), kind_pb(kd, 3), kind_pb(kd, 4), kind_pb(kd, 5)}};
}

__device__ __forceinline__ float f16_lo_back(unsigned u) {
    return (float)__builtin_bit_cast(f16x2, u)[0];
}
__device__ __forceinline__ float f16_hi_back(unsigned u) {
    return (float)__builtin_bit_cast(f16x2, u)[1];
}

template <bool F16>
__device__ __forceinline__ f32x16 mfma16(u32x4 a, u32x4 b, f32x16 c) {
    if constexpr (F16)
        return __builtin_amdgcn_mfma_f32_32x32x16_f16(__builtin_bit_cast(f16x8, a), __builtin_bit_cast(f16x8, b), c, 0, 0, 0);
    else
        return __builtin_amdgcn_mfma_f32_32x32x16_bf16(__builtin_bit_cast(bf16x8, a), __builtin_bit_cast(bf16x8, b), c, 0, 0, 0);
}

template <int KD>
__device__ __forceinline__ void split4(float4 v, uint2 (&out)[kind_parts_a(KD)]) {
    constexpr int NP = kind_parts_a(KD);
    if constexpr (kind_f16(KD)) {
        constexpr float FMAX = 65504.f;
        const float cx = __builtin_amdgcn_fmed3f(v.x, -FMAX, FMAX), cy = __builtin_amdgcn_fmed3f(v.y, -FMAX, FMAX);
        const float cz = __builtin_amdgcn_fmed3f(v.z, -FMAX, FMAX), cw = __builtin_amdgcn_fmed3f(v.w, -FMAX, FMAX);
        out[0] = make_uint2(pack_f16(cx, cy), pack_f16(cz, cw));
        if constexpr (NP == 2) {
            const unsigned lo = out[0].x, hi = out[0].y;
            out[1] = make_uint2(pack_f16(__builtin_amdgcn_fmed3f(v.x - f16_lo_back(lo), -FMAX, FMAX),
                                         __builtin_amdgcn_fmed3f(v.y - f16_hi_back(lo), -FMAX, FMAX)),
                                pack_f16(__builtin_amdgcn_fmed3f(v.z - f16_lo_back(hi), -FMAX, FMAX),
                                         __builtin_amdgcn_fmed3f(v.w - f16_hi_back(hi), -FMAX, FMAX)));
        }
        return;
    }
    float r[4] = {v.x, v.y, v.z, v.w};
#pragma unroll
    for (int p = 0; p < NP; ++p) {
        const unsigned lo = pack_bf16(r[0], r[1]), hi = pack_bf16(r[2], r[3]);
        out[p] = make_uint2(lo, hi);
        if (p + 1 < NP) {
            r[0] -= __builtin_bit_cast(float, lo << 16);
            r[1] -= __builtin_bit_cast(float, lo & 0xffff0000u);
            r[2] -= __builtin_bit_cast(float, hi << 16);
            r[3] -= __builtin_bit_cast(float, hi & 0xffff0000u);
        }
    }
}

__device__ __forceinline__ int weight_image_exp(const float* w_absmax) {
    if (!w_absmax) return 0;
    const float m = *w_absmax;
    int ex = 0;
    if (m > 0.f && m < 3.0e38f) (void)frexpf(m, &ex);
    const int t = ex + 3;
    return max(-120, min(120, 8 * (t >= 0 ? t / 8 : -((7 - t) / 8))));
}

__device__ __forceinline__ float style_range_guard(const float* styles, int cin, int lane, float* back,
                                                   const float* x_absmax, const float* w_absmax) {
    float m = styles ? 0.f : 1.f;
    if (styles)
        for (int i = lane; i < cin; i += 64) m = fmaxf(m, fabsf(styles[i]));
    float mx = x_absmax ? x_absmax[lane * HFAGP_ABSMAX_STRIDE] : 0.f;
#pragma unroll
    for (int o = 32; o > 0; o >>= 1) {
        m = fmaxf(m, __shfl_xor(m, o));
        mx = fmaxf(mx, __shfl_xor(mx, o));
    }
    int e = 0, ex = 15;
    if (m > 0.f && m < 3.0e38f) (void)frexpf(m, &e);
    if (mx > 0.f && mx < 3.0e38f) (void)frexpf(mx, &ex);
    e += ex - 15;
    e = max(-100, min(100, e));
    *back = ldexpf(1.f, max(-126, min(127, e + weight_image_exp(w_absmax))));
    return ldexpf(1.f, -e);
}

}

static inline int kind_of(int precision) {
    switch (precision) {
        case HFAGP_PREC_F16: return 1;
        case HFAGP_PREC_BF16X3: return 2;
        case HFAGP_PREC_BF16X6: return 3;
        case HFAGP_PREC_F16X3: return 4;
        case HFAGP_PREC_F16X2: return 5;
        default: return 0;
    }
}
```

hfa-gp_amd/csrc/torgb_skip.hip:

```cpp
#include "split_mfma.h"

namespace hfagp {

template <int KD, int TNC>
__global__ void __launch_bounds__(256, 3) torgb_skip_kernel(const HfagpTorgbSkipArgs a) {
    constexpr int NP = kind_parts(KD);
    constexpr bool F16 = kind_f16(KD);
    constexpr int NPROD = NP == 1 ? 1 : NP == 2 ? 3 : 6;
    constexpr int PA[6] = {0, 1, 0, 1, 2, 0};
    constexpr int PB[6] = {0, 0, 1, 1, 0, 2};
    __shared__ __attribute__((aligned(16))) float Ss[512];
    const int tid = threadIdx.x, lane = tid & 63, wave = tid >> 6, h = lane >> 5, l31 = lane & 31;
    const int HW = a.H * a.W;
    const long long pos0 = ((long long)blockIdx.x * 4 + wave) * 32;
    const int b = __builtin_amdgcn_readfirstlane((int)(((long long)blockIdx.x * 128) / HW));
    for (int i = tid; i < a.Cin; i += 256) Ss[i] = a.styles[(size_t)b * a.Cin + i];
    float sback = 1.f, sdown = 1.f;
    if constexpr (F16) sdown = style_range_guard(a.styles + (size_t)b * a.Cin, a.Cin, lane, &sback, a.x_absmax, a.w_absmax);
    __syncthreads();

    const int nchunks = a.Cin / CKB;
    const char* xl = reinterpret_cast<const char*>(a.x + (size_t)(pos0 + l31) * a.Cin + 8 * h);
    const char* wb = reinterpret_cast<const char*>(a.wt);
    const int cq8 = a.Cin >> 3;
    const long long part_stride = (long long)cq8 * a.Cout;
    unsigned bth[TNC];
#pragma unroll
    for (int tn = 0; tn < TNC; ++tn) bth[tn] = (unsigned)(h * a.Cout + tn * 32 + l31) * 16u;

    f32x16 acc[TNC];
#pragma unroll
    for (int tn = 0; tn < TNC; ++tn)
#pragma unroll
        for (int r = 0; r < 16; ++r) acc[tn][r] = 0.f;

    float4 xr[3][2];
    auto load_x = [&](int c, int slot) __attribute__((always_inline)) {
        const char* q = xl + (size_t)min(c, nchunks - 1) * (CKB * 4);
        xr[slot][0] = *reinterpret_cast<const float4*>(q);
        xr[slot][1] = *reinterpret_cast<const float4*>(q + 16);
    };
    u32x4 bq[TNC][NP];
    auto load_b = [&](int c) __attribute__((always_inline)) {
#pragma unroll
        for (int q = 0; q < NP; ++q) {
            const char* base = wb + (q * part_stride + (long long)c * 2 * a.Cout) * 16;
#pragma unroll
            for (int tn = 0; tn < TNC; ++tn) bq[tn][q] = *reinterpret_cast<const u32x4*>(base + bth[tn]);
        }
    };
    auto step = [&](int c, int slot) __attribute__((always_inline)) {
        load_b(c);
        const float4 s0 = *reinterpret_cast<const float4*>(Ss + c * CKB + 8 * h);
        const float4 s1 = *reinterpret_cast<const float4*>(Ss + c * CKB + 8 * h + 4);
        const float4 x0 = xr[slot][0], x1 = xr[slot][1];
        uint2 p0[NP], p1[NP];
        split4<KD>(make_float4(x0.x * (s0.x * sdown), x0.y * (s0.y * sdown), x0.z * (s0.z * sdown), x0.w * (s0.w * sdown)), p0);
        split4<KD>(make_float4(x1.x * (s1.x * sdown), x1.y * (s1.y * sdown), x1.z * (s1.z * sdown), x1.w * (s1.w * sdown)), p1);
        load_x(c + 3, slot);
        u32x4 af[NP];
#pragma unroll
        for (int q = 0; q < NP; ++q) af[q] = u32x4{p0[q].x, p0[q].y, p1[q].x, p1[q].y};
#pragma unroll
        for (int pr = 0; pr < NPROD; ++pr)
#pragma unroll
            for (int tn = 0; tn < TNC; ++tn) acc[tn] = mfma16<F16>(af[PA[pr]], bq[tn][PB[pr]], acc[tn]);
    };
    load_x(0, 0);
    load_x(1, 1);
    load_x(2, 2);
    int c = 0;
    for (; c + 3 <= nchunks; c += 3) {
        step(c, 0);
        step(c + 1, 1);
        step(c + 2, 2);
    }
    if (c < nchunks) step(c, 0);
    if (c + 1 < nchunks) step(c + 1, 1);

    const int pix0 = (int)(pos0 - (long long)b * HW);
    const int Y = pix0 / a.W, X0 = pix0 % a.W;
    const int Hi = a.H >> 1, Wi = a.W >> 1;
    int y0, y1; float wy0, wy1;
    up2_taps(Y, y0, y1, wy0, wy1);
    if (y0 < 0) { y0 = 0; wy0 = 0.f; }
    if (y1 >= Hi) { y1 = max(Hi - 1, 0); wy1 = 0.f; }
    float vmax = 0.f;
#pragma unroll
    for (int tn = 0; tn < TNC; ++tn) {
        const int co = tn * 32 + l31;
        const float bs = a.bias[co];
        float* dst = a.plane_major ? a.img_out + ((((size_t)b * 3 + tn) * a.H + Y) * a.W + X0) * 32 + l31
                                   : a.img_out + ((size_t)b * HW + pix0) * a.Cout + co;
        const int pstep = a.plane_major ? 32 : a.Cout;
        float o[16];
#pragma unroll
        for (int r = 0; r < 16; ++r) o[r] = fmaf(acc[tn][r], sback, bs);
        if (a.img_in) {
            const float* src0 = a.img_in + ((size_t)b * Hi + y0) * Wi * a.Cout + co;
            const float* src1 = a.img_in + ((size_t)b * Hi + y1) * Wi * a.Cout + co;
            float v0[4][4], v1[4][4];
#pragma unroll
            for (int g = 0; g < 4; ++g) {
                const int cb = (X0 >> 1) + 4 * g + 2 * h;
#pragma unroll
                for (int k = 0; k < 4; ++k) {
                    const int col = cb - 1 + k;
                    const int off = min(max(col, 0), Wi - 1) * a.Cout;
                    const bool in = col >= 0 && col < Wi;
                    const float t0 = src0[off], t1 = src1[off];
                    v0[g][k] = in ? t0 : 0.f;
                    v1[g][k] = in ? t1 : 0.f;
                }
            }
#pragma unroll
            for (int r = 0; r < 16; ++r) {
                const int g = r >> 2, q = r & 3;
                const int k0 = (q + 1) >> 1, k1 = k0 + 1;
                const float wx0 = (q & 1) ? 0.75f : 0.25f, wx1 = (q & 1) ? 0.25f : 0.75f;
                float t = o[r];
                t = fmaf(wy0 * wx0, v0[g][k0], t);
                t = fmaf(wy0 * wx1, v0[g][k1], t);
                t = fmaf(wy1 * wx0, v1[g][k0], t);
                t = fmaf(wy1 * wx1, v1[g][k1], t);
                o[r] = t;
            }
        }
#pragma unroll
        for (int r = 0; r < 16; ++r) {
            const int row = (r & 3) + 8 * (r >> 2) + 4 * h;
            dst[row * pstep] = o[r];
            vmax = fmaxf(vmax, fabsf(o[r]));
        }
    }
    if (a.out_absmax) publish_absmax(a.out_absmax, vmax, blockIdx.x * 4 + wave);
}

template <int KD>
static int launch_torgb_skip_kind(const HfagpTorgbSkipArgs* a, hipStream_t s) {
    const unsigned grid = (unsigned)(((long long)a->B * a->H * a->W) / 128);
    switch (a->Cout / 32) {
        case 1: torgb_skip_kernel<KD, 1><<<grid, 256, 0, s>>>(*a); break;
        case 2: torgb_skip_kernel<KD, 2><<<grid, 256, 0, s>>>(*a); break;
        case 3: torgb_skip_kernel<KD, 3><<<grid, 256, 0, s>>>(*a); break;
        default: torgb_skip_kernel<KD, 4><<<grid, 256, 0, s>>>(*a); break;
    }
    return check_launch("torgb_skip_fwd");
}

}

using namespace hfagp;

extern "C" int hfagp_torgb_skip_fwd(const HfagpTorgbSkipArgs* a, void* stream) {
    HFAGP_REQUIRE(a && a->x && a->wt && a->styles && a->bias && a->img_out, HFAGP_EBADARG, "torgb_skip: null pointer");
    HFAGP_REQUIRE(a->B > 0 && a->H > 0 && a->W > 0, HFAGP_EBADARG, "torgb_skip: bad dims");
    HFAGP_REQUIRE(a->Cout % 32 == 0 && a->Cout <= 128 && a->Cin % CKB == 0 && a->Cin <= 512 && a->W % 32 == 0 &&
                      (a->H * a->W) % 128 == 0 && (!a->img_in || (a->H % 2 == 0)),
                  HFAGP_EUNSUPPORTED, "torgb_skip: Cout=%d (multiple of 32, <= 128), Cin=%d (multiple of 16, <= 512), W=%d "
                                      "(multiple of 32), H*W=%d (multiple of 128); use hfagp_modconv_fwd + hfagp_skip_upsample_add",
                  a->Cout, a->Cin, a->W, a->H * a->W);
    HFAGP_REQUIRE(!a->plane_major || a->Cout == 96, HFAGP_EUNSUPPORTED, "torgb_skip: plane_major needs Cout = 96 (3 planes x 32)");
    hipStream_t s = (hipStream_t)stream;
    switch (kind_of(a->precision)) {
        case 1: return launch_torgb_skip_kind<1>(a, s);
        case 2: return launch_torgb_skip_kind<2>(a, s);
        case 3: return launch_torgb_skip_kind<3>(a, s);
        case 4: return launch_torgb_skip_kind<4>(a, s);
        case 5: return launch_torgb_skip_kind<4>(a, s);
        default: break;
    }
    set_error("torgb_skip: precision %d has no 16-bit weight image", a->precision);
    return HFAGP_EBADARG;
}
```

hfa-gp_amd/generator.py:

```python
from __future__ import annotations

import contextlib

import math
import os
from typing import Dict, Optional

import torch
from torch import nn

from . import ops
from .config import GeneratorConfig, ffhq512_128


class _Affine(nn.Module):
    def __init__(self, w_dim: int, cin: int, gen: torch.Generator):
        super().__init__()
        self.weight = nn.Parameter(torch.randn(cin, w_dim, generator=gen))
        self.bias = nn.Parameter(torch.ones(cin))


class _SynthesisLayer(nn.Module):
    def __init__(self, cin, cout, w_dim, resolution, up, taps, gen, use_noise=True):
        super().__init__()
# ... 338 lines not shown
        elif noise_mode != "none":
            raise NotImplementedError("noise_mode must be 'const' or 'none' (HFA-GP passes 'const', headnerf.py:112)")
        cout = layer.weight.shape[0]
        gain = math.sqrt(2.0)
        x_parts = 1 if self._precision_of(layer.weight) == "f16x2" else 0
        k_styles, k_dcoef = styles, dcoef
        flops = 2.0 * batch * x.shape[1] * x.shape[2] * x.shape[3] * cout * 9
        key = ("modconv" if wt.dtype == torch.float32 else
               "modconv_f16" if wt.dtype == torch.float16 and wt.shape[0] == 1 else "modconv_split")
        npos = x.shape[1] * x.shape[2]
        if (layer.up != 2 and wt.dtype != torch.float32 and npos <= 256 and x.shape[3] % 16 == 0
                and x.shape[3] <= 512 and cout % 32 == 0 and not half and rgb is None
                and not (npos >= 64 and batch * npos >= 1024)):
            key = "modconv_small"
        fuse = self.fuse_up_fir
        fuse = fuse in (True, "1") or (fuse == "auto" and x.shape[3] <= 64 and not half)
        if layer.up == 2 and fuse and ops.upconv_fir_supported(x, wt, cout, batch):
            def fused_layer():
                return self._timed(key + "_upfir", flops, ops.upconv_fir, x, wt, cout, k_styles, k_dcoef, noise, ns, layer.bias,
                                   "lrelu", cfg.lrelu_alpha, gain, conv_clamp, batch=batch, x_absmax=x_absmax,
                                   y_absmax=y_absmax, y_f16=half)
            out = self._timed(f"up_layer:{x.shape[3]}->{cout}@{2 * x.shape[1]}:fused", flops, fused_layer)
        elif layer.up == 2:
            def two_kernels():
                yt = self._timed(key + "_up", flops, ops.modconv, x, wt, cout, ops.CONVT3X3_UP2, styles=k_styles, batch=batch,
                                 x_absmax=x_absmax, y_f16=half, x_parts=x_parts)
                return ops.upfir_epilogue(yt, k_dcoef, noise, ns, layer.bias, "lrelu", cfg.lrelu_alpha, gain, conv_clamp,
                                          y_absmax=y_absmax)
            out = self._timed(f"up_layer:{x.shape[3]}->{cout}@{2 * x.shape[1]}", flops, two_kernels)
        else:
            rgb_w = None
            if rgb is not None and ops.fused_torgb_supported(x, wt, cout, batch):
                rgb_w = (rgb[1][:, None, :] * rgb[0][None]).contiguous()
            out = self._timed(key, flops, ops.modconv, x, wt, cout, ops.CONV3X3, styles=k_styles, dcoef=k_dcoef,
                              noise=noise, noise_strength=ns, bias=layer.bias, act="lrelu", alpha=cfg.lrelu_alpha,
                              gain=gain, clamp=conv_clamp, batch=batch, x_absmax=x_absmax, y_absmax=y_absmax,
                              rgb_w=rgb_w, y_f16=half, x_parts=x_parts,
                              store_y=keep_out or rgb_w is None or tape is not None or y_absmax is not None)
            if rgb_w is not None:
                out, self._rgb_part = out
        rec = None
        if tape is not None:
            rec = dict(layer=layer, x=x, styles=styles, dcoef=dcoef, out=out, row=row, up=layer.up, wsq=wsq,
                       producer=dict(dcoef=dcoef, bias=layer.bias, noise=noise_raw, noise_strength=ns if ns_dev is None else 0.0,
                                     noise_strength_dev=ns_dev, act="lrelu", alpha=cfg.lrelu_alpha, gain=gain, clamp=conv_clamp))
        return out, rec

    def _block(self, x, img, blk: _SynthesisBlock, ws, rows, batch, noise_mode, conv_clamp, small_rgb, last, tape,
               absmax=None, half=False, keep_out=True):
        rec = dict(conv0=None, first=blk.in_channels == 0, img_in=img, const=getattr(blk, "const", None))
        am_in, am0, am1 = absmax if absmax is not None else (None, None, None)
        tr = blk.torgb
        cin = tr.weight.shape[1]
        row = rows[-1]
        pre = self._styles.pop(id(tr), None) if self._styles else None
        styles = pre[0] if pre is not None else ops.styles_demod(ws[:, row], tr.affine.weight, tr.affine.bias, None,
                                                                 1.0 / math.sqrt(cin))[0]
        rgb = (tr.weight.detach().reshape(tr.weight.shape[0], cin), styles) if (small_rgb and tr.weight.shape[0] <= 3) else None
        self._rgb_part = None
        if blk.in_channels == 0:
            x, rec["conv1"] = self._layer(self._const(blk.const), blk.conv1, ws[:, rows[0]], rows[0], batch,
                                          noise_mode, conv_clamp, tape, None, am1, rgb)
        else:
            x, rec["conv0"] = self._layer(x, blk.conv0, ws[:, rows[0]], rows[0], batch, noise_mode, conv_clamp, tape,
                                          am_in, am0, None, half)
            x, rec["conv1"] = self._layer(x, blk.conv1, ws[:, rows[1]], rows[1], batch, noise_mode, conv_clamp, tape,
                                          am0, am1, rgb, half, keep_out)
        y = y_pre = None
        if small_rgb:
            if tape is not None and conv_clamp is not None:
                y_pre = torch.empty(batch, tr.weight.shape[0], x.shape[1], x.shape[2], device=x.device)
            if self._rgb_part is not None:
                img = ops.torgb_finish(self._rgb_part, tr.bias, img, conv_clamp, y_pre)
                self._rgb_part = None
            else:
                img = ops.torgb_small(x.float() if half else x, tr.weight.detach().reshape(tr.weight.shape[0], cin),
                                      styles, tr.bias, img, conv_clamp, y_pre)
        else:
            wt = self._gemm_image(tr.weight)
            side = self.side_stream(batch, x.device)
            main = torch.cuda.current_stream(x.device) if side is not None else None
            if side is not None:
                side.wait_stream(main)
                for t in (x, styles):
                    t.record_stream(side)
            with (torch.cuda.stream(side) if side is not None else contextlib.nullcontext()):
                self._planes_absmax = ops.absmax_slots(1, x.device)[0] if last else None
                if conv_clamp is None and x.shape[0] == batch and ops.torgb_skip_supported(x, wt, tr.weight.shape[0]):
                    img = ops.torgb_skip(x, wt, tr.weight.shape[0], styles, tr.bias, img, plane_major=last, x_absmax=am1,
                                         out_absmax=self._planes_absmax)
                else:
                    y = ops.modconv(x, wt, tr.weight.shape[0], ops.CONV1X1, styles=styles, bias=tr.bias, act="linear",
                                    gain=1.0, clamp=conv_clamp, batch=batch, x_absmax=am1)
                    img = ops.skip_upsample_add(img, y, plane_major=last, out_absmax=self._planes_absmax)
            if side is not None and last:
                main.wait_stream(side)
                img.record_stream(main)
                self._planes_absmax.record_stream(main)
        if tape is not None:
            rec["rgb"] = dict(torgb=tr, x=x, styles=styles, row=row, small=small_rgb, clamp=conv_clamp,
                              y=y if conv_clamp is not None else None, y_pre=y_pre)
            tape.append(rec)
        return x, img

    def _precompute_styles(self, ws: torch.Tensor, blocks_rows) -> None:
        cfg = self.cfg
        items, keys = [], []
        for blk, rows in blocks_rows:
            convs = [blk.conv1] if blk.in_channels == 0 else [blk.conv0, blk.conv1]
            for layer, row in zip(convs, rows):
                items.append((ws[:, row], layer.affine.weight, layer.affine.bias, self._prepared(layer.weight)[1], 1.0,
                              cfg.demod_eps))
                keys.append(id(layer))
            tr = blk.torgb
            items.append((ws[:, rows[-1]], tr.affine.weight, tr.affine.bias, None, 1.0 / math.sqrt(tr.weight.shape[1]),
                          cfg.demod_eps))
            keys.append(id(tr))
        self._styles = {}
        for i in range(0, len(items), 32):
            for k, v in zip(keys[i:i + 32], ops.styles_demod_batch(items[i:i + 32])):
                self._styles[k] = v

    def backbone_planes(self, ws: torch.Tensor, tape=None) -> torch.Tensor:
        if not getattr(self, "_in_forward", False):
            self._refresh_tuned(tape is not None)
        cfg = self.cfg
        syn = self.backbone.synthesis
        b = ws.shape[0]
        x = img = None
        idx = 0
        plan = []
        for res in cfg.block_resolutions:
            n_conv = 1 if res == 4 else 2
            plan.append((getattr(syn, f"b{res}"), list(range(idx, idx + n_conv + 1))))
            idx += n_conv
        self._precompute_styles(ws, plan)
        track = cfg.backbone_conv_clamp is None and (self._conv_precision in ("f16x3", "f16x2", "f16"))
        am = ops.absmax_slots(2 * len(cfg.block_resolutions), ws.device) if track else None
        self._absmax = (am, [f"b{res}.{c}" for res in cfg.block_resolutions for c in ("conv0", "conv1")]) if track else None
        idx = 0
        prev = None
        for k, res in enumerate(cfg.block_resolutions):
            blk = getattr(syn, f"b{res}")
            n_conv = 1 if res == 4 else 2
            rows = list(range(idx, idx + n_conv + 1))
            x, img = self._block(x, img, blk, ws, rows, b, cfg.backbone_noise_mode, cfg.backbone_conv_clamp, False,
                                 res == cfg.plane_resolution, tape,
                                 (prev, am[2 * k], am[2 * k + 1]) if track else None)
            prev = am[2 * k + 1] if track else None
            idx += n_conv
        side = self._side_streams.get(ws.device.index if ws.device.index is not None else torch.cuda.current_device())
        if side is not None and not torch.cuda.is_current_stream_capturing():
            torch.cuda.current_stream(ws.device).wait_stream(side)
        return img

    def f16_range_report(self) -> Optional[Dict[str, float]]:
        if getattr(self, "_absmax", None) is None:
            return None
        am, names = self._absmax
        vals = am.max(dim=1).values.tolist()
        return {n: v for n, v in zip(names, vals) if not n.startswith("b4.conv0")}

    def decoder_params(self):
        net = self.decoder.net
        return net["0"].weight, net["0"].bias, net["2"].weight, net["2"].bias

    def _render_args(self, c: torch.Tensor):
        cfg = self.cfg
# ... 444 lines not shown
```

hfa-gp_amd/ops.py:

```python
from __future__ import annotations

import ctypes as C
import math
import os
import types
from typing import Optional, Tuple

import torch

from . import _lib as L

CONV3X3, CONVT3X3_UP2, CONV1X1, CONV3X3_BWD, CONVS2_BWD = 0, 1, 2, 3, 4
ACT_LINEAR, ACT_LRELU = 0, 1
_ACT = {"linear": ACT_LINEAR, "lrelu": ACT_LRELU}


_raw_stream = getattr(torch._C, "_cuda_getCurrentRawStream", None)


def _stream() -> int:
    if _raw_stream is not None:
        return _raw_stream(torch.cuda.current_device())
    return torch.cuda.current_stream().cuda_stream

# ... 104 lines not shown
            else:
                dt = _IMAGE_DTYPE[pr]
                numel = NPARTS[pr] * kh * kw * ci * co
                sizes.append((dt, n16[dt], numel))
                n16[dt] += (numel + 256 + 7) // 8 * 8
        metas.append((sizes, nsq if want_wsq else None))
        if want_wsq:
            nsq += co * ci
    dev = items[0][0].device
    flat = {dt: torch.empty(n, device=dev, dtype=dt) for dt, n in n16.items() if n}
    sq = torch.empty(nsq, device=dev, dtype=torch.float32) if nsq else None
    amax = torch.empty(len(items), device=dev, dtype=torch.float32) if torch.float16 in flat else None
    out, arr = [], (L.WeightPrepItem * len(items))()
    for k, ((w, prec, prec_t, want_wsq), (sizes, sq_off)) in enumerate(zip(items, metas)):
        co, ci, kh, kw = w.shape
        views = []
        for pr, sz, shape in ((prec, sizes[0], (kh * kw, ci // 8, co, 8)), (prec_t, sizes[1], (kh * kw, co // 8, ci, 8))):
            if sz is None:
                views.append(None)
            else:
                dt, off, numel = sz
                views.append(flat[dt][off: off + numel].view(NPARTS[pr], *shape))
        wsq = sq[sq_off: sq_off + co * ci].view(co, ci) if want_wsq else None
        a = arr[k]
        a.weight = _ptr(w)
        a.image = views[0].data_ptr() if views[0] is not None else None
        a.image_t = views[1].data_ptr() if views[1] is not None else None
        a.wsq = _ptr(wsq)
        a.Cout, a.Cin, a.taps = co, ci, kh * kw
        a.precision = PRECISIONS[prec] if prec is not None else 0
        a.precision_t = PRECISIONS[prec_t] if prec_t is not None else 0
        for v in views:
            if v is not None and v.dtype == torch.float16:
                v.w_absmax = amax[k: k + 1]
                a.w_absmax = v.w_absmax.data_ptr()
        out.append((views[0], views[1], wsq))
    for k0 in range(0, len(items), 48):
        n = min(48, len(items) - k0)
        sub = (L.WeightPrepItem * n).from_buffer(arr, k0 * C.sizeof(L.WeightPrepItem))
        L.check(L.lib().hfagp_weight_prep_batch(sub, n, _stream()), "weight_prep_batch")
    return out


def weight_prep_split(weight: torch.Tensor, nparts: int) -> torch.Tensor:
    return _weight_prep_prec(weight, {1: "f16", 2: "bf16x3", 3: "bf16x6"}[nparts], scaled=False)


def _style_args(a, who: str, w, affine_w, affine_b, wsq, style_gain: float, eps: float):
    if w.dtype != torch.float32 or not w.is_cuda or w.stride(-1) != 1:
        raise RuntimeError(f"{who}: w must be a CUDA fp32 tensor with unit inner stride")
    if w.dim() != 2 or affine_w.dim() != 2:
        raise RuntimeError(f"{who}: w must be [B, w_dim] and affine_w [Cin, w_dim], got {list(w.shape)} and {list(affine_w.shape)}")
    b, wd = w.shape
    cin = affine_w.shape[0]
    _chk_operand(who, "affine_w", affine_w, (cin, wd), w)
    _chk_operand(who, "affine_b", affine_b, (cin,), w)
    if wsq is not None:
        if wsq.dim() != 2:
            raise RuntimeError(f"{who}: wsq must be [Cout, Cin], got {list(wsq.shape)}")
        _chk_operand(who, "wsq", wsq, (wsq.shape[0], cin), w)
    styles = torch.empty(b, cin, device=w.device, dtype=torch.float32)
    dcoef = None
    a.w, a.affine_w, a.affine_b = _ptr(w), _ptr(affine_w), _ptr(affine_b)
    a.styles = _ptr(styles)
    a.B, a.w_dim, a.w_stride, a.Cin = b, wd, w.stride(0), cin
    a.style_gain, a.eps = style_gain, eps
    if wsq is not None:
        dcoef = torch.empty(b, wsq.shape[0], device=w.device, dtype=torch.float32)
        a.wsq, a.dcoef, a.Cout = _ptr(wsq), _ptr(dcoef), wsq.shape[0]
    return styles, dcoef


def styles_demod(w: torch.Tensor, affine_w: torch.Tensor, affine_b: torch.Tensor,
                 wsq: Optional[torch.Tensor], style_gain: float = 1.0, eps: float = 1e-8):
    a = L.StyleArgs()
    out = _style_args(a, "styles_demod", w, affine_w, affine_b, wsq, style_gain, eps)
    L.check(L.lib().hfagp_style_fwd(C.byref(a), _stream()), "style_fwd")
    return out


def styles_demod_batch(items):
    arr = (L.StyleArgs * len(items))()
    out = [_style_args(a, "styles_demod_batch", *item) for a, item in zip(arr, items)]
    L.check(L.lib().hfagp_style_batch_fwd(arr, len(items), _stream()), "style_batch_fwd")
    return out


def qr_gram(gram: torch.Tensor, top: torch.Tensor) -> Tuple[torch.Tensor, torch.Tensor]:
    n = gram.shape[0]
    r = torch.empty(n, n, device=gram.device, dtype=torch.float32)
    rinv = torch.empty(n, n, device=gram.device, dtype=torch.float32)
    L.check(L.lib().hfagp_qr_gram_fwd(_ptr(_chk(gram, "gram")), _ptr(_chk(top, "top")), _ptr(r), _ptr(rinv), n, _stream()),
            "qr_gram_fwd")
    return r, rinv


def qr_refine(gram: torch.Tensor, status: Optional[torch.Tensor] = None) -> Tuple[torch.Tensor, torch.Tensor]:
    n = gram.shape[0]
    r = torch.empty(n, n, device=gram.device, dtype=torch.float32)
    rinv = torch.empty(n, n, device=gram.device, dtype=torch.float32)
    L.check(L.lib().hfagp_qr_refine_fwd(_ptr(_chk(gram, "gram")), _ptr(r), _ptr(rinv), _ptr(status), n, _stream()),
            "qr_refine_fwd")
    return r, rinv


def tall_gram(x: torch.Tensor, y: torch.Tensor, scale: float = 1.0) -> torch.Tensor:
    m, n = x.shape
    for t in (x, y):
        if t.shape != (m, n) or t.dtype != torch.float32 or not t.is_cuda or 1 not in (t.stride(0), t.stride(1)):
            raise RuntimeError("tall_gram: operands must be fp32 device matrices of one shape with a unit stride")
    out = torch.empty(n, n, device=x.device, dtype=torch.float32)
    ws = torch.empty(L.lib().hfagp_tall_gram_workspace_bytes(m, n) // 4, device=x.device, dtype=torch.float32)
    L.check(L.lib().hfagp_tall_gram(x.data_ptr(), x.stride(0), x.stride(1), y.data_ptr(), y.stride(0), y.stride(1), _ptr(ws),
                                    _ptr(out), m, n, scale, _stream()), "tall_gram")
    return out


class TallSkinnyQR(torch.autograd.Function):

    @staticmethod
    def forward(ctx, a: torch.Tensor, status: Optional[torch.Tensor] = None) -> torch.Tensor:
        n = a.shape[1]
        gram = tall_gram(a, a)
        _, rinv1 = qr_gram(gram, a[:n, :n].contiguous())
        q1 = a @ rinv1
        _, rinv2 = qr_refine(tall_gram(q1, q1), status)
        rinv = rinv1 @ rinv2
        q = q1 @ rinv2
        ctx.save_for_backward(q, rinv)
        return q

    @staticmethod
    def backward(ctx, gq: torch.Tensor):
        q, rinv = ctx.saved_tensors
        if gq.stride(0) != 1 and gq.stride(1) != 1:
            gq = gq.contiguous()
        x = torch.triu(tall_gram(q, gq, -1.0))
        s = x + x.T - torch.diag(torch.diagonal(x))
        return (gq + q @ s) @ rinv.T, None


def fully_connected(x: torch.Tensor, weight: torch.Tensor, bias: Optional[torch.Tensor], lr_mul: float = 1.0,
                    act: str = "linear", alpha: float = 0.2, gain: Optional[float] = None) -> torch.Tensor:
    _chk(x, "x")
    b, fin = x.shape
    fout = weight.shape[0]
    if gain is None:
        gain = math.sqrt(2.0) if act == "lrelu" else 1.0
    y = torch.empty(b, fout, device=x.device, dtype=torch.float32)
    L.check(L.lib().hfagp_fc_fwd(_ptr(x), _ptr(_chk(weight, "weight")), _ptr(bias), _ptr(y), b, fin, fout, lr_mul,
                                 _ACT[act], alpha, gain, _stream()), "fc_fwd")
    return y


def absmax_slots(n: int, device) -> torch.Tensor:
    return torch.zeros(n, L.ABSMAX_FLOATS, device=device, dtype=torch.float32)


_IMAGE_PRECISION = {(torch.float16, 1): PREC_F16, (torch.float16, 2): PREC_F16X3,
                    (torch.bfloat16, 2): PREC_BF16X3, (torch.bfloat16, 3): PREC_BF16X6}


def _image_precision(wt: torch.Tensor, x_parts: int = 0, who: str = "modconv") -> int:
    if wt.dtype == torch.float32:
        return PREC_F32
    prec = _IMAGE_PRECISION.get((wt.dtype, wt.shape[0])) if wt.dim() == 5 else None
    if prec is None:
        raise RuntimeError(f"{who}: 16-bit weight images must come from weight_prep_prec")
    if x_parts == 1 and prec != PREC_F16:
        if prec != PREC_F16X3:
            raise RuntimeError(f"{who}: x_parts=1 ('f16x2') goes with the two-part float16 weight image")
        prec = PREC_F16X2
    return prec


def _modconv_args(x: torch.Tensor, wt: torch.Tensor, cout: int, mode: int, styles=None, dcoef=None, noise=None,
                  noise_strength: float = 0.0, bias=None, act: str = "linear", alpha: float = 0.2, gain: float = 1.0,
                  clamp: Optional[float] = None, batch: Optional[int] = None, ksplit: int = 0, x_absmax=None, y_absmax=None,
                  rgb_w=None, y_f16: bool = False, x_parts: int = 0, who: str = "modconv"):
    if mode == CONVS2_BWD:
        _, _, xb, h, w, cin = x.shape
        h, w = h - 1, w - 1
    else:
        xb, h, w, cin = x.shape
    b = batch if batch is not None else xb
    a = L.ModconvArgs()
    a.x, a.wt, a.precision = x.data_ptr(), wt.data_ptr(), _image_precision(wt, x_parts, who)
    a.styles, a.dcoef, a.noise, a.bias = _ptr(styles), _ptr(dcoef), _ptr(noise), _ptr(bias)
    a.x_batch_stride = 0 if (xb == 1 and b > 1) else x.shape[-3] * x.shape[-2] * cin
    a.B, a.H, a.W, a.Cin, a.Cout = b, h, w, cin, cout
    a.mode, a.act, a.ksplit = mode, _ACT[act], ksplit
    a.noise_strength, a.alpha, a.gain, a.clamp = noise_strength, alpha, gain, _clamp(clamp)
    a.x_absmax, a.y_absmax, a.rgb_w = _ptr(x_absmax), _ptr(y_absmax), _ptr(rgb_w)
    a.x_f16, a.y_f16 = int(x.dtype == torch.float16), int(y_f16)
    a.w_absmax = _ptr(getattr(wt, "w_absmax", None))
    return a, b, h, w


def modconv(x: torch.Tensor, wt: torch.Tensor, cout: int, mode: int, styles: Optional[torch.Tensor] = None,
            dcoef: Optional[torch.Tensor] = None, noise: Optional[torch.Tensor] = None, noise_strength: float = 0.0,
            bias: Optional[torch.Tensor] = None, act: str = "linear", alpha: float = 0.2, gain: float = 1.0,
            clamp: Optional[float] = None, batch: Optional[int] = None, ksplit: int = 0, x_absmax: Optional[torch.Tensor] = None,
            y_absmax: Optional[torch.Tensor] = None, rgb_w: Optional[torch.Tensor] = None, y_f16: bool = False,
            store_y: bool = True, x_parts: int = 0):
    if (x.dtype == torch.float16 or y_f16) and not (wt.dtype == torch.float16 and wt.dim() == 5 and wt.shape[0] == 1):
        raise RuntimeError("modconv: fp16 storage (float16 x / y_f16) goes with the single-pass fp16 weight image")
    _chk_act(x, "x")
    if wt.dtype == torch.float32:
        _chk(wt, "wt")
    elif not (wt.is_cuda and wt.is_contiguous()):
        raise RuntimeError("modconv: 16-bit weight images must come from weight_prep_prec")
    if rgb_w is not None:
        _chk(rgb_w, "rgb_w")
    a, b, h, w = _modconv_args(x, wt, cout, mode, styles, dcoef, noise, noise_strength, bias, act, alpha, gain, clamp, batch,
                               ksplit, x_absmax, y_absmax, rgb_w, y_f16, x_parts)
    ydt = torch.float16 if y_f16 else torch.float32
    if not store_y:
        if rgb_w is None or y_absmax is not None:
            raise RuntimeError("modconv: store_y=False needs rgb_w (the fused toRGB is then the only output) and no y_absmax")
        y = None
    elif mode == CONVT3X3_UP2:
        y = torch.empty(b, 2 * h + 1, 2 * w + 1, cout, device=x.device, dtype=ydt)
    else:
        y = torch.empty(b, h, w, cout, device=x.device, dtype=ydt)
    a.y = _ptr(y)
    nbytes = L.lib().hfagp_modconv_workspace_bytes(C.byref(a))
    ws = torch.empty(nbytes // 4, device=x.device, dtype=torch.float32) if nbytes else None
    part = None
    if rgb_w is not None:
        part = torch.empty(L.lib().hfagp_modconv_rgb_parts(C.byref(a)), b, h, w, 4, device=x.device, dtype=torch.float32)
    a.workspace, a.rgb_part = _ptr(ws), _ptr(part)
    L.check(L.lib().hfagp_modconv_fwd(C.byref(a), _stream()), "modconv_fwd")
    return y if rgb_w is None else (y, part)


_PLAN_UNSPLIT = {}
_NONNULL = 1


def _plan_unsplit(key, build, rgb: bool = False) -> bool:
    r = _PLAN_UNSPLIT.get(key)
    if r is None:
        a = build()
        a.x, a.wt, a.y, a.rgb_w = a.x or _NONNULL, a.wt or _NONNULL, _NONNULL, _NONNULL if rgb else None
        r = _PLAN_UNSPLIT[key] = L.lib().hfagp_modconv_workspace_bytes(C.byref(a)) == 0
    return r


def f16_storage_supported(h: int, w: int, cin: int, cout: int, batch: int) -> bool:
    if cin % 16 != 0 or cout % 128 != 0:
        return False

    def call(mode):
        x = torch.empty(batch, h, w, cin, dtype=torch.float16, device="meta")
        wt = torch.empty(1, 9, cin // 8, cout, 8, dtype=torch.float16, device="meta")
        return _modconv_args(x, wt, cout, mode, y_f16=True)[0]
    return all(_plan_unsplit((mode, batch, h, w, cin, cout, PREC_F16, 1, 1, False, False), lambda: call(mode))
               for mode in (CONV3X3, CONVT3X3_UP2))


def fused_torgb_supported(x: torch.Tensor, wt: torch.Tensor, cout: int, batch: int) -> bool:
    if wt.dtype == torch.float32 or cout % 128 != 0:
        return False
    xb, h, w, cin = x.shape
    key = (CONV3X3, batch, h, w, cin, cout, _image_precision(wt), int(x.dtype == torch.float16), 0, True, xb == 1 and batch > 1)
    return _plan_unsplit(key, lambda: _modconv_args(x, wt, cout, CONV3X3, batch=batch)[0], rgb=True)


def torgb_finish(part: torch.Tensor, bias: torch.Tensor, rgb_in: Optional[torch.Tensor], clamp: Optional[float],
                 y_pre: Optional[torch.Tensor] = None) -> torch.Tensor:
    _chk(part, "part")
    if part.dim() != 5 or part.shape[4] != 4 or bias.dim() != 1:
        raise RuntimeError(f"torgb_finish: part must be [nparts, B, H, W, 4] and bias [Cout], got {list(part.shape)} and {list(bias.shape)}")
    nparts, b, h, w, _ = part.shape
    cout = bias.shape[0]
    _chk_operand("torgb_finish", "bias", bias, (cout,), part)
    _chk_operand("torgb_finish", "rgb_in", rgb_in, (b, cout, h // 2, w // 2), part)
    _chk_operand("torgb_finish", "y_pre", y_pre, (b, cout, h, w), part)
    out = torch.empty(b, cout, h, w, device=part.device, dtype=torch.float32)
    a = L.TorgbFinishArgs()
    a.part, a.bias, a.rgb_out, a.y_pre = _ptr(part), _ptr(bias), _ptr(out), _ptr(y_pre)
    a.rgb_in = _ptr(rgb_in)
    a.nparts, a.B, a.H, a.W, a.Cout = nparts, b, h, w, cout
    a.clamp = _clamp(clamp)
    L.check(L.lib().hfagp_torgb_finish_fwd(C.byref(a), _stream()), "torgb_finish_fwd")
    return out


_FIR_SCRATCH = {}
_FIR_RETIRED = []
_FIR_BYTES = {}


def _fir_scratch_bytes(a) -> int:
    key = (a.B, a.H, a.W, a.Cin, a.Cout, a.precision, a.x_f16, a.x_batch_stride == 0,
           os.environ.get("HFAGP_DEV_FIR_MIN_BLOCKS"), os.environ.get("HFAGP_DEV_FIR_NSEG"), os.environ.get("HFAGP_DEV_FIR_LEAN"))
    n = _FIR_BYTES.get(key)
    if n is None:
        n = _FIR_BYTES[key] = int(L.lib().hfagp_upconv_fir_scratch_bytes(C.byref(a)))
    return n


def upconv_fir_supported(x: torch.Tensor, wt: torch.Tensor, cout: int, batch: Optional[int] = None) -> bool:
    if wt.dtype == torch.float32 or not x.is_cuda or (x.dtype == torch.float16 and not (wt.dtype == torch.float16 and wt.shape[0] == 1)):
        return False
    a, *_ = _modconv_args(x, wt, cout, CONVT3X3_UP2, batch=batch, who="upconv_fir")
    return _fir_scratch_bytes(a) > 0


def upconv_fir(x: torch.Tensor, wt: torch.Tensor, cout: int, styles: Optional[torch.Tensor], dcoef: Optional[torch.Tensor],
               noise: Optional[torch.Tensor], noise_strength: float, bias: Optional[torch.Tensor], act: str = "lrelu",
               alpha: float = 0.2, gain: float = math.sqrt(2.0), clamp: Optional[float] = None, batch: Optional[int] = None,
               x_absmax: Optional[torch.Tensor] = None, y_absmax: Optional[torch.Tensor] = None,
               y_f16: bool = False) -> torch.Tensor:
    _chk_act(x, "x")
# ... 10 lines not shown
        if scratch is not None:
            _FIR_RETIRED.append(scratch)
        grown = 1 << max(nbytes - 1, 1).bit_length()
        scratch = _FIR_SCRATCH[key] = torch.empty(grown // 4, device=x.device, dtype=torch.float32)
    y = torch.empty(b, 2 * h, 2 * w, cout, device=x.device, dtype=torch.float16 if y_f16 else torch.float32)
    a.y = y.data_ptr()
    L.check(L.lib().hfagp_upconv_fir_fwd(C.byref(a), _ptr(scratch), _stream()), "upconv_fir_fwd")
    return y


def upfir_epilogue(yt: torch.Tensor, dcoef: Optional[torch.Tensor], noise: Optional[torch.Tensor],
                   noise_strength: float, bias: Optional[torch.Tensor], act: str = "lrelu", alpha: float = 0.2,
                   gain: float = math.sqrt(2.0), clamp: Optional[float] = None,
                   y_absmax: Optional[torch.Tensor] = None) -> torch.Tensor:
    half = _chk_act(yt, "yt").dtype == torch.float16
    if yt.dim() != 4 or yt.shape[1] < 3 or yt.shape[2] < 3 or yt.shape[1] % 2 == 0 or yt.shape[2] % 2 == 0:
        raise RuntimeError(f"upfir_epilogue: yt must be [B, 2H+1, 2W+1, C] with an odd height and width of at least 3, got {list(yt.shape)}")
    b, hi, wi, c = yt.shape
    h, w = (hi - 1) // 2, (wi - 1) // 2
    _chk_operand("upfir_epilogue", "dcoef", dcoef, (b, c), yt)
    _chk_operand("upfir_epilogue", "noise", noise, (2 * h, 2 * w), yt)
    _chk_operand("upfir_epilogue", "bias", bias, (c,), yt)
    _chk_absmax("upfir_epilogue", "y_absmax", y_absmax, yt)
    y = torch.empty(b, 2 * h, 2 * w, c, device=yt.device, dtype=yt.dtype)
    a = L.UpfirEpilogueArgs()
    a.yt, a.dcoef, a.noise, a.bias, a.y = yt.data_ptr(), _ptr(dcoef), _ptr(noise), _ptr(bias), y.data_ptr()
    a.io_f16 = int(half)
    a.B, a.H, a.W, a.C, a.act = b, h, w, c, _ACT[act]
    a.noise_strength, a.alpha, a.gain = noise_strength, alpha, gain
    a.clamp = _clamp(clamp)
    a.y_absmax = _ptr(y_absmax)
    L.check(L.lib().hfagp_upfir_epilogue_fwd(C.byref(a), _stream()), "upfir_epilogue_fwd")
    return y


def skip_upsample_add(img: Optional[torch.Tensor], y: torch.Tensor, plane_major: bool = False,
                      out_absmax: Optional[torch.Tensor] = None) -> torch.Tensor:
    _chk(y, "y")
    if y.dim() != 4:
        raise RuntimeError(f"skip_upsample_add: y must be [B, H, W, C], got {list(y.shape)}")
    b, ho, wo, c = y.shape
    _chk_absmax("skip_upsample_add", "out_absmax", out_absmax, y)
    a = L.SkipArgs()
    if img is not None:
        if ho % 2 or wo % 2:
            raise RuntimeError(f"skip_upsample_add: y {list(y.shape)} must have an even height and width to add an up-sampled img to")
        _chk_operand("skip_upsample_add", "img", img, (b, ho // 2, wo // 2, c), y)
        a.img_in, a.H, a.W = _ptr(img), img.shape[1], img.shape[2]
    else:
        a.H, a.W = ho, wo
    out = torch.empty((b, 3, ho, wo, c // 3) if plane_major else (b, ho, wo, c), device=y.device,
                      dtype=torch.float32)
    a.y, a.img_out, a.B, a.C, a.plane_major = _ptr(y), _ptr(out), b, c, int(plane_major)
    a.out_absmax = _ptr(out_absmax)
    L.check(L.lib().hfagp_skip_upsample_add(C.byref(a), _stream()), "skip_upsample_add")
    return out


def torgb_skip_supported(x: torch.Tensor, wt: torch.Tensor, cout: int) -> bool:
    b, h, w, cin = x.shape
    return (wt.dtype in (torch.float16, torch.bfloat16) and cout % 32 == 0 and cout <= 128 and cin % 16 == 0 and
            cin <= 512 and w % 32 == 0 and (h * w) % 128 == 0 and b * h * w >= 512 * 32)


def torgb_skip(x: torch.Tensor, wt: torch.Tensor, cout: int, styles: torch.Tensor, bias: torch.Tensor,
               img: Optional[torch.Tensor], plane_major: bool = False, x_absmax: Optional[torch.Tensor] = None,
               out_absmax: Optional[torch.Tensor] = None) -> torch.Tensor:
    _chk(x, "x")
    b, h, w, cin = x.shape
    if not (wt.is_cuda and wt.is_contiguous() and wt.dim() == 5 and wt.dtype in (torch.float16, torch.bfloat16)):
        raise RuntimeError("torgb_skip: the weight image must come from weight_prep_prec (16-bit kinds)")
    a = L.TorgbSkipArgs()
    a.precision = _image_precision(wt, who="torgb_skip")
    out = torch.empty((b, 3, h, w, cout // 3) if plane_major else (b, h, w, cout), device=x.device, dtype=torch.float32)
    a.x, a.wt, a.styles, a.bias = _ptr(x), wt.data_ptr(), _ptr(_chk(styles, "styles")), _ptr(_chk(bias, "bias"))
    if img is not None:
        _chk(img, "img")
        if img.shape != (b, h // 2, w // 2, cout):
            raise RuntimeError(f"torgb_skip: img {tuple(img.shape)} is not the half-resolution image of {(b, h, w, cout)}")
        a.img_in = _ptr(img)
    a.img_out, a.x_absmax, a.out_absmax = _ptr(out), _ptr(x_absmax), _ptr(out_absmax)
    a.w_absmax = _ptr(getattr(wt, "w_absmax", None))
    a.B, a.H, a.W, a.Cin, a.Cout, a.plane_major = b, h, w, cin, cout, int(plane_major)
    L.check(L.lib().hfagp_torgb_skip_fwd(C.byref(a), _stream()), "torgb_skip_fwd")
    return out


def torgb_small(x: torch.Tensor, weight: torch.Tensor, styles: torch.Tensor, bias: torch.Tensor,
                rgb_in: Optional[torch.Tensor], clamp: Optional[float], y_pre: Optional[torch.Tensor] = None) -> torch.Tensor:
    _chk(x, "x")
    if x.dim() != 4 or weight.dim() != 2:
        raise RuntimeError(f"torgb_small: x must be [B, H, W, Cin] and weight [Cout, Cin], got {list(x.shape)} and {list(weight.shape)}")
    b, h, w, cin = x.shape
    cout = weight.shape[0]
    _chk_operand("torgb_small", "weight", weight, (cout, cin), x)
    _chk_operand("torgb_small", "styles", styles, (b, cin), x)
    _chk_operand("torgb_small", "bias", bias, (cout,), x)
    _chk_operand("torgb_small", "rgb_in", rgb_in, (b, cout, h // 2, w // 2), x)
    _chk_operand("torgb_small", "y_pre", y_pre, (b, cout, h, w), x)
    out = torch.empty(b, cout, h, w, device=x.device, dtype=torch.float32)
    a = L.TorgbArgs()
    a.y_pre = _ptr(y_pre)
    a.x, a.weight, a.styles, a.bias = _ptr(x), _ptr(weight), _ptr(styles), _ptr(bias)
    a.rgb_in = _ptr(rgb_in)
    a.rgb_out = _ptr(out)
    a.B, a.H, a.W, a.Cin, a.Cout = b, h, w, cin, cout
    a.clamp = _clamp(clamp)
    L.check(L.lib().hfagp_torgb_fwd(C.byref(a), _stream()), "torgb_fwd")
    return out


_DEC = ("dec_w0", "dec_b0", "dec_w1", "dec_b1")


def _planes_dims(who: str, planes: torch.Tensor):
    _chk(planes, f"{who}: planes")
    if planes.dim() != 5 or planes.shape[1] != 3 or planes.shape[4] != 32:
        raise RuntimeError(f"{who}: planes must be [B, 3, H, W, 32]")
    return planes.shape[0], planes.shape[2], planes.shape[3]


def _plane_axes_id(plane_axes) -> int:
    if isinstance(plane_axes, str):
        return 0 if plane_axes == "eg3d_original" else 1
    return plane_axes


def _fill_decoder(who: str, a, planes: torch.Tensor, params, decoder_precision: str, planes_absmax) -> None:
    for name, t in zip(_DEC, params):
        setattr(a, name, _ptr(_chk(t, f"{who}: {name}")))
    a.planes_absmax = _ptr(_decoder_bound(planes, decoder_precision, planes_absmax)) if planes.numel() else None


def _ray_args(who: str, f, planes, cam2world, intrinsics, u_strat, u_imp, dec_w0, dec_b0, dec_w1, dec_b1, res: int, ray_start: float,
              ray_end: float, box_warp: float, decoder_lr_mul: float, plane_axes, white_back: bool, decoder_precision: str, planes_absmax,
              state):
    b, h, w = _planes_dims(who, planes)
    r = res * res
    sc, sf = u_strat.shape[-1], u_imp.shape[-1]
    if u_strat.numel() != b * r * sc or u_imp.numel() != b * r * sf:
        raise RuntimeError(f"{who}: u_strat / u_imp have the wrong number of elements")
    if state is not None and _chk(state, f"{who}: state").shape != (b, r, (sc + sf) * 35):
        raise RuntimeError(f"{who}: state must be [B, R, {(sc + sf) * 35}] (raymarch_state), got {tuple(state.shape)}")
    for name, t in (("cam2world", cam2world), ("intrinsics", intrinsics), ("u_strat", u_strat), ("u_imp", u_imp)):
        setattr(f, name, _ptr(_chk(t, f"{who}: {name}")))
    f.planes, f.state = _ptr(planes), _ptr(state)
    _fill_decoder(who, f, planes, (dec_w0, dec_b0, dec_w1, dec_b1), decoder_precision, planes_absmax)
    f.B, f.H, f.W, f.res, f.Sc, f.Sf = b, h, w, res, sc, sf
    f.plane_axes, f.white_back = _plane_axes_id(plane_axes), int(white_back)
    f.ray_start, f.ray_end, f.box_warp, f.decoder_lr_mul = ray_start, ray_end, box_warp, decoder_lr_mul
    return b, h, w, r, sc, sf


def _dec_grad_out(who: str, a, params, decoder_grads: bool, dec_out):
    if not decoder_grads:
        return None
    dec = tuple(dec_out) if dec_out is not None else tuple(torch.zeros_like(t) for t in params)
    if len(dec) != 4 or any(t.shape != like.shape or t.dtype != torch.float32 or not t.is_contiguous() or not t.is_cuda
                            for t, like in zip(dec, params)):
        raise RuntimeError(f"{who}: dec_out must be four contiguous fp32 device tensors shaped like the decoder parameters")
    a.d_dec_w0, a.d_dec_b0, a.d_dec_w1, a.d_dec_b1 = (_ptr(t) for t in dec)
    return dec


def _query_points(who: str, coords: torch.Tensor, b: int) -> int:
    _chk(coords, f"{who}: coords")
    if coords.dim() != 3 or coords.shape[2] != 3 or coords.shape[0] not in (1, b):
# ... 829 lines not shown
```

include/hfagp.h:

```cpp
#ifndef HFAGP_H_
#define HFAGP_H_

#include <stddef.h>
#include <stdint.h>

#ifdef __cplusplus
extern "C" {
#endif

#define HFAGP_ABI_VERSION 15

enum { HFAGP_OK = 0, HFAGP_EBADARG = -1, HFAGP_EUNSUPPORTED = -2, HFAGP_ELAUNCH = -3 };

int hfagp_abi_version(void);
const char* hfagp_last_error(void);

#define HFAGP_RAYMARCH_STATE_FLOATS_PER_SAMPLE 35

typedef struct {
    const float* planes;
    const float* cam2world;
    const float* intrinsics;
    const float* u_strat;
    const float* u_imp;
// ... 37 lines not shown
    const float* dec_w1;
    const float* dec_b1;
    const float* planes_absmax;
    float*       sigma;
    float*       rgb;
    int64_t M;
    int64_t out_stride;
    int32_t B, H, W;
    int32_t Bc;
    int32_t N;
    int32_t x_begin, x_count;
    int32_t plane_axes;
    float decoder_lr_mul;
    double box_warp;
    double cube_length;
} HfagpPlanesQueryArgs;

int hfagp_planes_query(const HfagpPlanesQueryArgs* a, void* stream);

typedef struct {
    const float* planes;
    const float* coords;
    const float* dec_w0;
    const float* dec_b0;
    const float* dec_w1;
    const float* dec_b1;
    const float* planes_absmax;
    const float* g_sigma;
    const float* g_rgb;
    float*       d_planes;
    float*       d_coords;
    float*       d_dec_w0;
    float*       d_dec_b0;
    float*       d_dec_w1;
    float*       d_dec_b1;
    int64_t M;
    int32_t B, H, W;
    int32_t Bc;
    int32_t plane_axes;
    float decoder_lr_mul;
    double box_warp;
} HfagpPlanesQueryBwdArgs;

int hfagp_planes_query_bwd(const HfagpPlanesQueryBwdArgs* a, void* stream);

int hfagp_planes_query_normals(const HfagpPlanesQueryArgs* a, float* grad ,
                               float* normal , void* stream);

int hfagp_planes_query_normals_bwd(const HfagpPlanesQueryBwdArgs* a ,
                                   const float* g_grad, const float* g_normal, void* stream);

typedef struct {
    const float* volume;
    void*        workspace;
    int64_t*     counts;
    float*       verts;
    int32_t*     faces;
    int64_t workspace_bytes;
    int64_t vert_capacity;
    int64_t face_capacity;
    int32_t n0, n1, n2;
    float level;
    float origin[3];
    float spacing[3];
} HfagpMarchingCubesArgs;

size_t hfagp_marching_cubes_workspace_bytes(int32_t n0, int32_t n1, int32_t n2);
int hfagp_marching_cubes_count(const HfagpMarchingCubesArgs* a, void* stream);
int hfagp_marching_cubes_emit(const HfagpMarchingCubesArgs* a, void* stream);

typedef struct {
    const float* w;
    const float* affine_w;
    const float* affine_b;
    const float* wsq;
    float*       styles;
    float*       dcoef;
    int32_t B, w_dim, w_stride, Cin, Cout;
    float style_gain, eps;
} HfagpStyleArgs;

int hfagp_style_fwd(const HfagpStyleArgs* a, void* stream);
int hfagp_style_batch_fwd(const HfagpStyleArgs* items, int32_t n, void* stream);

int hfagp_qr_gram_fwd(const float* gram, const float* top, float* R, float* Rinv, int32_t n, void* stream);
int hfagp_qr_refine_fwd(const float* gram, float* R, float* Rinv, float* status, int32_t n, void* stream);
size_t hfagp_tall_gram_workspace_bytes(int32_t m, int32_t n);
int hfagp_tall_gram(const float* X, int64_t x_rs, int64_t x_cs, const float* Y, int64_t y_rs, int64_t y_cs, float* workspace,
                    float* out, int32_t m, int32_t n, float scale, void* stream);

int hfagp_fc_fwd(const float* x, const float* weight, const float* bias, float* y, int32_t B, int32_t In, int32_t Out,
                 float lr_mul, int32_t act, float alpha, float gain, void* stream);

int hfagp_weight_prep(const float* weight, float* wt, float* wsq,
                      int32_t Cout, int32_t Cin, int32_t taps, void* stream);

int hfagp_weight_prep_split(const float* weight, void* wb, int32_t Cout, int32_t Cin, int32_t taps,
                            int32_t nparts, void* stream);
int hfagp_weight_prep_prec(const float* weight, void* wb, int32_t Cout, int32_t Cin, int32_t taps,
                           int32_t precision, void* stream);
int hfagp_weight_prep_scaled(const float* weight, void* wb, float* w_absmax, int32_t Cout, int32_t Cin, int32_t taps,
                             int32_t precision, void* stream);

typedef struct {
    const float* weight;
    void*        image;
    void*        image_t;
    float*       wsq;
    int32_t Cout, Cin, taps;
    int32_t precision, precision_t;
    float*       w_absmax;
} HfagpWeightPrepItem;
int hfagp_weight_prep_batch(const HfagpWeightPrepItem* items, int32_t n, void* stream);

enum {
    HFAGP_CONV3X3 = 0,
    HFAGP_CONVT3X3_UP2 = 1,
    HFAGP_CONV1X1 = 2,
    HFAGP_CONV3X3_BWD = 3,
    HFAGP_CONVS2_BWD = 4
};
enum { HFAGP_ACT_LINEAR = 0, HFAGP_ACT_LRELU = 1 };
enum { HFAGP_PREC_F32 = 0, HFAGP_PREC_BF16X3 = 1, HFAGP_PREC_BF16X6 = 2, HFAGP_PREC_F16 = 3, HFAGP_PREC_F16X3 = 4,
       HFAGP_PREC_F16X2 = 5 };

typedef struct {
    const float* x;
    const void*  wt;
    const float* styles;
    const float* dcoef;
    const float* noise;
    const float* bias;
    float*       y;
    float*       workspace;
    int64_t x_batch_stride;
    int32_t B, H, W, Cin, Cout;
    int32_t mode, act;
    int32_t ksplit;
    float noise_strength, alpha, gain, clamp;
    int32_t precision;
    const float* x_absmax;
    float*       y_absmax;
    const float* rgb_w;
    float*       rgb_part;
    int32_t x_f16, y_f16;
    const float* w_absmax;
} HfagpModconvArgs;
int32_t hfagp_modconv_rgb_parts(const HfagpModconvArgs* a);
#define HFAGP_ABSMAX_SLOTS 64
#define HFAGP_ABSMAX_STRIDE 32
#define HFAGP_ABSMAX_FLOATS (HFAGP_ABSMAX_SLOTS * HFAGP_ABSMAX_STRIDE)

size_t hfagp_modconv_workspace_bytes(const HfagpModconvArgs* a);
int hfagp_modconv_fwd(const HfagpModconvArgs* a, void* stream);

typedef struct {
    const void*  yt;
    const float* dcoef;
    const float* noise;
    const float* bias;
    void*        y;
    int32_t B, H, W, C;
    int32_t act;
    float noise_strength, alpha, gain, clamp;
    float*       y_absmax;
    int32_t      io_f16;
} HfagpUpfirEpilogueArgs;

int hfagp_upfir_epilogue_fwd(const HfagpUpfirEpilogueArgs* a, void* stream);

size_t hfagp_upconv_fir_scratch_bytes(const HfagpModconvArgs* a);
int hfagp_upconv_fir_fwd(const HfagpModconvArgs* a, void* scratch, void* stream);

typedef struct {
    const float* img_in;
    const float* y;
    float*       img_out;
    int32_t B, H, W, C;
    int32_t plane_major;
    float*       out_absmax;
} HfagpSkipArgs;

int hfagp_skip_upsample_add(const HfagpSkipArgs* a, void* stream);

typedef struct {
    const float* x;
    const void*  wt;
    const float* styles;
    const float* bias;
    const float* img_in;
    float*       img_out;
    const float* x_absmax;
    float*       out_absmax;
    int32_t B, H, W, Cin, Cout;
    int32_t precision;
    int32_t plane_major;
    const float* w_absmax;
} HfagpTorgbSkipArgs;

int hfagp_torgb_skip_fwd(const HfagpTorgbSkipArgs* a, void* stream);

typedef struct {
    const float* x;
    const float* weight;
    const float* styles;
    const float* bias;
    const float* rgb_in;
    float*       rgb_out;
    float*       y_pre;
    int32_t B, H, W, Cin, Cout;
    float clamp;
} HfagpTorgbArgs;

int hfagp_torgb_fwd(const HfagpTorgbArgs* a, void* stream);

typedef struct {
    const float* part;
    const float* bias;
    const float* rgb_in;
    float*       rgb_out;
    float*       y_pre;
    int32_t nparts, B, H, W, Cout;
    float clamp;
} HfagpTorgbFinishArgs;
int hfagp_torgb_finish_fwd(const HfagpTorgbFinishArgs* a, void* stream);


typedef struct {
    const float* dxs_conv;
    const float* s_conv;
    const float* dxs_rgb;
    const float* s_rgb;
    const float* g_rgb_small;
    const float* w_rgb_small;
    const float* s_small;
    const float* g_direct;
    const float* x;
    const float* dcoef_p;
    const float* bias_p;
    const float* noise_p;
    float*       g_out;
    float*       partial;
    float*       sums;
    int32_t B, H, W, C, Co, nchunks, has_producer, act_p, param_grads;
    float noise_strength_p, alpha, gain, clamp;
    const float* y_rgb_small;
    const float* g_nchw3_a;
    const float* g_nchw3_b;
    float clamp_rgb_small;
    const float* noise_strength_dev;
} HfagpPointwiseBwdArgs;

int hfagp_pointwise_bwd(const HfagpPointwiseBwdArgs* a, void* stream);

typedef struct {
    const float* partial;
    float*       sums;
    int32_t B, nchunks, n;
} HfagpReducePartialsItem;
int hfagp_reduce_partials_batch(const HfagpReducePartialsItem* items, int32_t n, void* stream);

int hfagp_depth_clamp(float* depth, const float* tminmax, int64_t n, void* stream);

int hfagp_upfir_bwd(const float* gy, float* gph, int32_t B, int32_t H, int32_t W, int32_t C, void* stream);

int hfagp_upsample2d_bwd(const float* g, float* gin, int64_t outer, int32_t H, int32_t W, int32_t inner, void* stream);

int hfagp_planes_to_nhwc(const float* pm, float* y, int32_t B, int32_t H, int32_t W, int32_t Cp, void* stream);

typedef struct {
    const float* ds;
    const float* dd;
    const float* styles;
    const float* dcoef;
    const float* wsq;
    const float* affine_w;
    float*       dstot;
    float*       dw;
    int32_t B, Cin, Cout, w_dim, dw_stride, accumulate;
    float style_gain;
} HfagpStyleBwdArgs;

int hfagp_style_bwd(const HfagpStyleBwdArgs* a, void* stream);
// ... 121 lines not shown
```

Before: 1030 frames/s.

## Precompute per-sample style absmax once and reuse it in conv range guards

The batched demod kernel now also computes each sample's style absmax into a small table, attached to the styles tensor. The modconv (merged-upsample path) and torgb_skip kernels read this table instead of each block re-reducing a full style row to find its range. The x/w absmax loads are issued early and reduced with DPP, and torgb now prefetches x chunks before the guard. This costs an extra small allocation and host-side pointer setup per style batch, and adds a legacy env switch.

```diff
diff --git a/hfa-gp_amd/_lib.py b/hfa-gp_amd/_lib.py
--- a/hfa-gp_amd/_lib.py
+++ b/hfa-gp_amd/_lib.py
@@ -196,6 +196,9 @@
     "hfagp_tall_gram": (C.c_int, [C.c_void_p, C.c_int64, C.c_int64, C.c_void_p, C.c_int64, C.c_int64, C.c_void_p, C.c_void_p,
                                   C.c_int32, C.c_int32, C.c_float, C.c_void_p]),
     "hfagp_style_batch_fwd": (C.c_int, [C.POINTER(StyleArgs), C.c_int32, C.c_void_p]),
+    "hfagp_style_batch_absmax_fwd": (C.c_int, [C.POINTER(StyleArgs), C.POINTER(C.c_void_p), C.c_int32, C.c_void_p]),
+    "hfagp_modconv_guard_fwd": (C.c_int, [C.POINTER(ModconvArgs), C.c_void_p, C.c_void_p]),
+    "hfagp_torgb_skip_guard_fwd": (C.c_int, [C.POINTER(TorgbSkipArgs), C.c_void_p, C.c_void_p]),
     "hfagp_weight_prep_split": (C.c_int, [C.c_void_p, C.c_void_p, C.c_int32, C.c_int32, C.c_int32, C.c_int32, C.c_void_p]),
     "hfagp_weight_prep_prec": (C.c_int, [C.c_void_p, C.c_void_p, C.c_int32, C.c_int32, C.c_int32, C.c_int32, C.c_void_p]),
     "hfagp_weight_prep_scaled": (C.c_int, [C.c_void_p, C.c_void_p, C.c_void_p, C.c_int32, C.c_int32, C.c_int32, C.c_int32, C.c_void_p]),
diff --git a/hfa-gp_amd/csrc/elementwise.hip b/hfa-gp_amd/csrc/elementwise.hip
--- a/hfa-gp_amd/csrc/elementwise.hip
+++ b/hfa-gp_amd/csrc/elementwise.hip
@@ -44,7 +44,7 @@
 }
 
 constexpr int kStyleBatch = 32;
-struct StyleBatch { HfagpStyleArgs it[kStyleBatch]; };
+struct StyleBatch { HfagpStyleArgs it[kStyleBatch]; float* amax[kStyleBatch]; };
 
 __global__ void __launch_bounds__(256) style_batch_kernel(const StyleBatch t) {
     const HfagpStyleArgs& a = t.it[blockIdx.y];
@@ -66,10 +66,19 @@
 
 __global__ void __launch_bounds__(256) demod_batch_kernel(const StyleBatch t) {
     const HfagpStyleArgs& a = t.it[blockIdx.y];
-    if (!a.dcoef) return;
+    float* amax = t.amax[blockIdx.y];
     const int wave = (blockIdx.x * blockDim.x + threadIdx.x) >> 6;
     const int lane = threadIdx.x & 63;
-    if (wave >= a.B * a.Cout) return;
+    const int nd = a.dcoef ? a.B * a.Cout : 0;
+    if (wave >= nd) {
+        if (!amax || wave >= nd + a.B) return;
+        const float* s = a.styles + (size_t)(wave - nd) * a.Cin;
+        float m = 0.f;
+        for (int k = lane; k < a.Cin; k += 64) m = fmaxf(m, fabsf(s[k]));
+        for (int o = 32; o > 0; o >>= 1) m = fmaxf(m, __shfl_xor(m, o));
+        if (lane == 0) amax[wave - nd] = m;
+        return;
+    }
     const int b = wave / a.Cout, o = wave % a.Cout;
     const float* s = a.styles + (size_t)b * a.Cin;
     const float* q = a.wsq + (size_t)o * a.Cin;
@@ -549,7 +558,7 @@
     return check_launch("style_fwd");
 }
 
-int hfagp_style_batch_fwd(const HfagpStyleArgs* items, int32_t n, void* stream) {
+static int style_batch_fwd(const HfagpStyleArgs* items, float* const* style_absmax, int32_t n, void* stream) {
     HFAGP_REQUIRE(items && n >= 1 && n <= kStyleBatch, HFAGP_EBADARG, "style_batch_fwd: 1..%d items, got %d", kStyleBatch, n);
     StyleBatch t;
     int max_s = 0, max_d = 0;
@@ -560,13 +569,23 @@
                       "style_batch_fwd: bad dims in item %d: B=%d Cin=%d w_dim=%d", i, a.B, a.Cin, a.w_dim);
         HFAGP_REQUIRE(!a.dcoef || (a.wsq && a.Cout > 0), HFAGP_EBADARG, "style_batch_fwd: item %d: dcoef without wsq", i);
         t.it[i] = a;
+        t.amax[i] = style_absmax ? style_absmax[i] : nullptr;
         max_s = a.B * a.Cin > max_s ? a.B * a.Cin : max_s;
-        if (a.dcoef) max_d = a.B * a.Cout > max_d ? a.B * a.Cout : max_d;
-    }
+        const int nd = (a.dcoef ? a.B * a.Cout : 0) + (t.amax[i] ? a.B : 0);
+        max_d = nd > max_d ? nd : max_d;
+    }
+    for (int i = n; i < kStyleBatch; ++i) t.amax[i] = nullptr;
     hipStream_t s = (hipStream_t)stream;
     style_batch_kernel<<<dim3((max_s + 3) / 4, n), 256, 0, s>>>(t);
     if (max_d) demod_batch_kernel<<<dim3((max_d + 3) / 4, n), 256, 0, s>>>(t);
     return check_launch("style_batch_fwd");
+}
+
+int hfagp_style_batch_fwd(const HfagpStyleArgs* items, int32_t n, void* stream) { return style_batch_fwd(items, nullptr, n, stream); }
+
+int hfagp_style_batch_absmax_fwd(const HfagpStyleArgs* items, float* const* style_absmax, int32_t n, void* stream) {
+    HFAGP_REQUIRE(style_absmax, HFAGP_EBADARG, "style_batch_absmax_fwd: null pointer");
+    return style_batch_fwd(items, style_absmax, n, stream);
 }
 
 int hfagp_fc_fwd(const float* x, const float* weight, const float* bias, float* y, int32_t B, int32_t In, int32_t Out,
diff --git a/hfa-gp_amd/csrc/modconv.hip b/hfa-gp_amd/csrc/modconv.hip
--- a/hfa-gp_amd/csrc/modconv.hip
+++ b/hfa-gp_amd/csrc/modconv.hip
@@ -1,4 +1,5 @@
 #include "modconv_plan.h"
+#include "split_mfma.h"
 
 namespace hfagp {
 
@@ -255,11 +256,12 @@
 
 int32_t hfagp_modconv_rgb_parts(const HfagpModconvArgs* a) { return a ? ((a->Cout + 127) / 128) * 2 : 0; }
 
-int hfagp_modconv_fwd(const HfagpModconvArgs* a, void* stream) {
+static int modconv_fwd(const HfagpModconvArgs* a, const float* style_absmax, void* stream) {
     Plan pl;
     int rc = resolve_modconv(a, pl);
     if (rc != HFAGP_OK) return rc;
     ConvParams& p = pl.p;
+    p.style_absmax = pl.merged_up ? guard_table(style_absmax, a->styles) : nullptr;
     HFAGP_REQUIRE((a->rgb_w == nullptr) == (a->rgb_part == nullptr), HFAGP_EBADARG, "modconv: rgb_w and rgb_part go together");
     if (pl.small) {
         rc = launch_smallconv(a, pl, (hipStream_t)stream);
@@ -313,4 +315,10 @@
     return rc;
 }
 
-}
+int hfagp_modconv_fwd(const HfagpModconvArgs* a, void* stream) { return modconv_fwd(a, nullptr, stream); }
+
+int hfagp_modconv_guard_fwd(const HfagpModconvArgs* a, const float* style_absmax, void* stream) {
+    return modconv_fwd(a, style_absmax, stream);
+}
+
+}
diff --git a/hfa-gp_amd/csrc/modconv_bf16.hip b/hfa-gp_amd/csrc/modconv_bf16.hip
--- a/hfa-gp_amd/csrc/modconv_bf16.hip
+++ b/hfa-gp_amd/csrc/modconv_bf16.hip
@@ -448,6 +448,8 @@
     char* As = lds_raw;
     float* Ss = reinterpret_cast<float*>(lds_raw + 2 * A_BUF);
 
+    GuardLoads gl;
+    if constexpr (F16) gl.issue(p.x_absmax, p.w_absmax, threadIdx.x & 63);
     unsigned id = p.xcd ? xcd_remap(blockIdx.x, gridDim.x) : blockIdx.x;
     const int tiles_nu = p.Cout / BNU;
     const int tn_blk = __builtin_amdgcn_readfirstlane(id % tiles_nu);  id /= tiles_nu;
@@ -475,12 +477,18 @@
     {
         const long long s_lo = (long long)b_lo * p.Cin, s_n = (long long)p.B * p.Cin;
         for (int i = tid; i < p.up_ns * p.Cin; i += NTH) Ss[i] = (p.styles && s_lo + i < s_n) ? p.styles[s_lo + i] : 1.f;
-        for (int sI = 0; sI < p.up_ns; ++sI) {
-            float bk = 1.f, dn = 1.f;
-            if constexpr (F16)
-                dn = style_range_guard((p.styles && b_lo + sI < p.B) ? p.styles + (size_t)(b_lo + sI) * p.Cin : nullptr, p.Cin, lane, &bk,
-                                       p.x_absmax, p.w_absmax);
-            if (tid == 0) { Gd[sI] = dn; Gd[p.up_ns + sI] = bk; }
+        if (F16 && p.style_absmax) {
+            float bk = 1.f;
+            const float dn = gl.scales((lane < p.up_ns && b_lo + lane < p.B) ? p.style_absmax[b_lo + lane] : 1.f, &bk);
+            if (tid < p.up_ns) { Gd[tid] = dn; Gd[p.up_ns + tid] = bk; }
+        } else {
+            for (int sI = 0; sI < p.up_ns; ++sI) {
+                float bk = 1.f, dn = 1.f;
+                if constexpr (F16)
+                    dn = style_range_guard((p.styles && b_lo + sI < p.B) ? p.styles + (size_t)(b_lo + sI) * p.Cin : nullptr, p.Cin, lane, &bk,
+                                           p.x_absmax, p.w_absmax);
+                if (tid == 0) { Gd[sI] = dn; Gd[p.up_ns + sI] = bk; }
+            }
         }
     }
     __syncthreads();
@@ -1013,6 +1021,8 @@
     char* As = lds_raw;
     float* Ss = reinterpret_cast<float*>(lds_raw + 2 * A_BUF);
 
+    GuardLoads gl;
+    gl.issue(p.x_absmax, p.w_absmax, threadIdx.x & 63);
     unsigned id = p.xcd ? xcd_remap(blockIdx.x, gridDim.x) : blockIdx.x;
     const int tiles_nu = p.Cout / 64;
     const int tn_blk = __builtin_amdgcn_readfirstlane(id % tiles_nu);  id /= tiles_nu;
@@ -1033,12 +1043,35 @@
     const int c_end = __builtin_amdgcn_readfirstlane((int)(((long long)nch * (ks + 1)) / p.ksplit));
 
     float* Gb = Ss + p.up_ns * p.Cin;
-    for (int sI = 0; sI < p.up_ns; ++sI) {
-        const float* st = (p.styles && b_lo + sI < p.B) ? p.styles + (size_t)(b_lo + sI) * p.Cin : nullptr;
-        float bk = 1.f;
-        const float dn = style_range_guard(st, p.Cin, lane, &bk, p.x_absmax, p.w_absmax);
-        for (int i = tid; i < p.Cin; i += 256) Ss[sI * p.Cin + i] = (st ? st[i] : 1.f) * dn;
-        if (tid == 0) Gb[sI] = bk;
+    float smaxv = 1.f, sv[2][2];
+    auto load_rows = [&](int s0) __attribute__((always_inline)) {
+#pragma unroll
+        for (int j = 0; j < 2; ++j)
+#pragma unroll
+            for (int k = 0; k < 2; ++k)
+                sv[j][k] = (b_lo + s0 + j < p.B && s0 + j < p.up_ns && tid + 256 * k < p.Cin)
+                               ? p.styles[(size_t)(b_lo + s0 + j) * p.Cin + tid + 256 * k] : 1.f;
+    };
+    auto store_rows = [&](int s0, float dnv) __attribute__((always_inline)) {
+#pragma unroll
+        for (int j = 0; j < 2; ++j) {
+            const float dn = __builtin_bit_cast(float, __builtin_amdgcn_readlane(__builtin_bit_cast(int, dnv), min(s0 + j, p.up_ns - 1)));
+#pragma unroll
+            for (int k = 0; k < 2; ++k)
+                if (s0 + j < p.up_ns && tid + 256 * k < p.Cin) Ss[(s0 + j) * p.Cin + tid + 256 * k] = sv[j][k] * dn;
+        }
+    };
+    if (p.style_absmax) {
+        if (lane < p.up_ns && b_lo + lane < p.B) smaxv = p.style_absmax[b_lo + lane];
+        load_rows(0);
+    } else {
+        for (int sI = 0; sI < p.up_ns; ++sI) {
+            const float* st = (p.styles && b_lo + sI < p.B) ? p.styles + (size_t)(b_lo + sI) * p.Cin : nullptr;
+            float bk = 1.f;
+            const float dn = style_range_guard(st, p.Cin, lane, &bk, p.x_absmax, p.w_absmax);
+            for (int i = tid; i < p.Cin; i += 256) Ss[sI * p.Cin + i] = (st ? st[i] : 1.f) * dn;
+            if (tid == 0) Gb[sI] = bk;
+        }
     }
 
     const int nsamp = min(p.up_ns, p.B - b_lo);
@@ -1064,6 +1097,13 @@
         sels |= (unsigned)sel << (14 + 3 * k);
     }
     static_assert((8 * (3 + 4 * (A_PER_T - 1)) + 7) * 16 < OCT, "every slot lies inside its octet");
+    if (p.style_absmax) {
+        float bkv = 1.f;
+        const float dnv = gl.scales(smaxv, &bkv);
+        store_rows(0, dnv);
+        for (int s0 = 2; s0 < p.up_ns; s0 += 2) { load_rows(s0); store_rows(s0, dnv); }
+        if (tid < p.up_ns) Gb[tid] = bkv;
+    }
     float4 ra[2];
     auto load_a = [&](int chunk, auto part_tag) __attribute__((always_inline)) {
         constexpr int PT = decltype(part_tag)::value;
diff --git a/hfa-gp_amd/csrc/modconv_plan.h b/hfa-gp_amd/csrc/modconv_plan.h
--- a/hfa-gp_amd/csrc/modconv_plan.h
+++ b/hfa-gp_amd/csrc/modconv_plan.h
@@ -37,6 +37,7 @@
     int xcd;
     int act; float noise_strength, alpha, gain, clamp;
     Phase phase[4];
+    const float* style_absmax;
 };
 
 struct Plan {
diff --git a/hfa-gp_amd/csrc/split_mfma.h b/hfa-gp_amd/csrc/split_mfma.h
--- a/hfa-gp_amd/csrc/split_mfma.h
+++ b/hfa-gp_amd/csrc/split_mfma.h
@@ -1,4 +1,5 @@
 #pragma once
+#include <cstdlib>
 #include "common.h"
 
 namespace hfagp {
@@ -81,13 +82,22 @@
     }
 }
 
-__device__ __forceinline__ int weight_image_exp(const float* w_absmax) {
-    if (!w_absmax) return 0;
-    const float m = *w_absmax;
+__device__ __forceinline__ int weight_image_exp_of(float m) {
     int ex = 0;
     if (m > 0.f && m < 3.0e38f) (void)frexpf(m, &ex);
     const int t = ex + 3;
     return max(-120, min(120, 8 * (t >= 0 ? t / 8 : -((7 - t) / 8))));
+}
+__device__ __forceinline__ int weight_image_exp(const float* w_absmax) { return w_absmax ? weight_image_exp_of(*w_absmax) : 0; }
+
+__device__ __forceinline__ float range_guard_scales(float m, float mx, int ew, float* back) {
+    int e = 0, ex = 15;
+    if (m > 0.f && m < 3.0e38f) (void)frexpf(m, &e);
+    if (mx > 0.f && mx < 3.0e38f) (void)frexpf(mx, &ex);
+    e += ex - 15;
+    e = max(-100, min(100, e));
+    *back = ldexpf(1.f, max(-126, min(127, e + ew)));
+    return ldexpf(1.f, -e);
 }
 
 __device__ __forceinline__ float style_range_guard(const float* styles, int cin, int lane, float* back,
@@ -101,15 +111,45 @@
         m = fmaxf(m, __shfl_xor(m, o));
         mx = fmaxf(mx, __shfl_xor(mx, o));
     }
-    int e = 0, ex = 15;
-    if (m > 0.f && m < 3.0e38f) (void)frexpf(m, &e);
-    if (mx > 0.f && mx < 3.0e38f) (void)frexpf(mx, &ex);
-    e += ex - 15;
-    e = max(-100, min(100, e));
-    *back = ldexpf(1.f, max(-126, min(127, e + weight_image_exp(w_absmax))));
-    return ldexpf(1.f, -e);
+    return range_guard_scales(m, mx, weight_image_exp(w_absmax), back);
 }
 
+template <int CTRL>
+__device__ __forceinline__ float dpp_max(float v) {
+    return fmaxf(v, __builtin_bit_cast(float, __builtin_amdgcn_update_dpp(0, __builtin_bit_cast(int, v), CTRL, 0xf, 0xf, false)));
+}
+__device__ __forceinline__ float wave_max(float v) {
+    v = dpp_max<0xB1>(v);
+    v = dpp_max<0x4E>(v);
+    v = dpp_max<0x141>(v);
+    v = dpp_max<0x140>(v);
+    const float r0 = __builtin_bit_cast(float, __builtin_amdgcn_readlane(__builtin_bit_cast(int, v), 0));
+    const float r1 = __builtin_bit_cast(float, __builtin_amdgcn_readlane(__builtin_bit_cast(int, v), 16));
+    const float r2 = __builtin_bit_cast(float, __builtin_amdgcn_readlane(__builtin_bit_cast(int, v), 32));
+    const float r3 = __builtin_bit_cast(float, __builtin_amdgcn_readlane(__builtin_bit_cast(int, v), 48));
+    return fmaxf(fmaxf(r0, r1), fmaxf(r2, r3));
+}
+
+struct GuardLoads {
+    float slot;
+    float wmax;
+    __device__ __forceinline__ void issue(const float* x_absmax, const float* w_absmax, int lane) {
+        slot = x_absmax ? x_absmax[lane * HFAGP_ABSMAX_STRIDE] : 0.f;
+        wmax = w_absmax ? *w_absmax : 0.f;
+    }
+    __device__ __forceinline__ float scales(float m, float* back) const {
+        return range_guard_scales(m, wave_max(slot), weight_image_exp_of(wmax), back);
+    }
+};
+__device__ __forceinline__ float guard_style_max(const float* style_absmax, bool has_styles, int b) {
+    return has_styles ? style_absmax[b] : 1.f;
+}
+
+}
+
+static inline const float* guard_table(const float* style_absmax, const float* styles) {
+    const char* dev = getenv("HFAGP_DEV_GUARD_LEGACY");
+    return (dev && atoi(dev) == 1) || !styles ? nullptr : style_absmax;
 }
 
 static inline int kind_of(int precision) {
diff --git a/hfa-gp_amd/csrc/torgb_skip.hip b/hfa-gp_amd/csrc/torgb_skip.hip
--- a/hfa-gp_amd/csrc/torgb_skip.hip
+++ b/hfa-gp_amd/csrc/torgb_skip.hip
@@ -3,7 +3,7 @@
 namespace hfagp {
 
 template <int KD, int TNC>
-__global__ void __launch_bounds__(256, 3) torgb_skip_kernel(const HfagpTorgbSkipArgs a) {
+__global__ void __launch_bounds__(256, 3) torgb_skip_kernel(const HfagpTorgbSkipArgs a, const float* style_absmax) {
     constexpr int NP = kind_parts(KD);
     constexpr bool F16 = kind_f16(KD);
     constexpr int NPROD = NP == 1 ? 1 : NP == 2 ? 3 : 6;
@@ -14,13 +14,34 @@
     const int HW = a.H * a.W;
     const long long pos0 = ((long long)blockIdx.x * 4 + wave) * 32;
     const int b = __builtin_amdgcn_readfirstlane((int)(((long long)blockIdx.x * 128) / HW));
-    for (int i = tid; i < a.Cin; i += 256) Ss[i] = a.styles[(size_t)b * a.Cin + i];
+    GuardLoads gl;
+    if constexpr (F16) gl.issue(a.x_absmax, a.w_absmax, lane);
+    const float* srow = a.styles + (size_t)b * a.Cin;
+    const float smax = (F16 && style_absmax) ? style_absmax[b] : 0.f;
+    float sv[2];
+#pragma unroll
+    for (int k = 0; k < 2; ++k) sv[k] = tid + 256 * k < a.Cin ? srow[tid + 256 * k] : 0.f;
+    const int nchunks = a.Cin / CKB;
+    const char* xl = reinterpret_cast<const char*>(a.x + (size_t)(pos0 + l31) * a.Cin + 8 * h);
+    float4 xr[3][2];
+    auto load_x = [&](int c, int slot) __attribute__((always_inline)) {
+        const char* q = xl + (size_t)min(c, nchunks - 1) * (CKB * 4);
+        xr[slot][0] = *reinterpret_cast<const float4*>(q);
+        xr[slot][1] = *reinterpret_cast<const float4*>(q + 16);
+    };
+    if constexpr (F16) {
+        load_x(0, 0);
+        load_x(1, 1);
+        load_x(2, 2);
+    }
     float sback = 1.f, sdown = 1.f;
-    if constexpr (F16) sdown = style_range_guard(a.styles + (size_t)b * a.Cin, a.Cin, lane, &sback, a.x_absmax, a.w_absmax);
+    if constexpr (F16)
+        sdown = style_absmax ? gl.scales(smax, &sback) : style_range_guard(srow, a.Cin, lane, &sback, a.x_absmax, a.w_absmax);
+#pragma unroll
+    for (int k = 0; k < 2; ++k)
+        if (tid + 256 * k < a.Cin) Ss[tid + 256 * k] = sv[k];
     __syncthreads();
 
-    const int nchunks = a.Cin / CKB;
-    const char* xl = reinterpret_cast<const char*>(a.x + (size_t)(pos0 + l31) * a.Cin + 8 * h);
     const char* wb = reinterpret_cast<const char*>(a.wt);
     const int cq8 = a.Cin >> 3;
     const long long part_stride = (long long)cq8 * a.Cout;
@@ -34,12 +55,6 @@
 #pragma unroll
         for (int r = 0; r < 16; ++r) acc[tn][r] = 0.f;
 
-    float4 xr[3][2];
-    auto load_x = [&](int c, int slot) __attribute__((always_inline)) {
-        const char* q = xl + (size_t)min(c, nchunks - 1) * (CKB * 4);
-        xr[slot][0] = *reinterpret_cast<const float4*>(q);
-        xr[slot][1] = *reinterpret_cast<const float4*>(q + 16);
-    };
     u32x4 bq[TNC][NP];
     auto load_b = [&](int c) __attribute__((always_inline)) {
 #pragma unroll
@@ -66,9 +81,11 @@
 #pragma unroll
             for (int tn = 0; tn < TNC; ++tn) acc[tn] = mfma16<F16>(af[PA[pr]], bq[tn][PB[pr]], acc[tn]);
     };
-    load_x(0, 0);
-    load_x(1, 1);
-    load_x(2, 2);
+    if constexpr (!F16) {
+        load_x(0, 0);
+        load_x(1, 1);
+        load_x(2, 2);
+    }
     int c = 0;
     for (; c + 3 <= nchunks; c += 3) {
         step(c, 0);
@@ -137,13 +154,13 @@
 }
 
 template <int KD>
-static int launch_torgb_skip_kind(const HfagpTorgbSkipArgs* a, hipStream_t s) {
+static int launch_torgb_skip_kind(const HfagpTorgbSkipArgs* a, const float* style_absmax, hipStream_t s) {
     const unsigned grid = (unsigned)(((long long)a->B * a->H * a->W) / 128);
     switch (a->Cout / 32) {
-        case 1: torgb_skip_kernel<KD, 1><<<grid, 256, 0, s>>>(*a); break;
-        case 2: torgb_skip_kernel<KD, 2><<<grid, 256, 0, s>>>(*a); break;
-        case 3: torgb_skip_kernel<KD, 3><<<grid, 256, 0, s>>>(*a); break;
-        default: torgb_skip_kernel<KD, 4><<<grid, 256, 0, s>>>(*a); break;
+        case 1: torgb_skip_kernel<KD, 1><<<grid, 256, 0, s>>>(*a, style_absmax); break;
+        case 2: torgb_skip_kernel<KD, 2><<<grid, 256, 0, s>>>(*a, style_absmax); break;
+        case 3: torgb_skip_kernel<KD, 3><<<grid, 256, 0, s>>>(*a, style_absmax); break;
+        default: torgb_skip_kernel<KD, 4><<<grid, 256, 0, s>>>(*a, style_absmax); break;
     }
     return check_launch("torgb_skip_fwd");
 }
@@ -152,7 +169,7 @@
 
 using namespace hfagp;
 
-extern "C" int hfagp_torgb_skip_fwd(const HfagpTorgbSkipArgs* a, void* stream) {
+static int torgb_skip_fwd(const HfagpTorgbSkipArgs* a, const float* style_absmax, void* stream) {
     HFAGP_REQUIRE(a && a->x && a->wt && a->styles && a->bias && a->img_out, HFAGP_EBADARG, "torgb_skip: null pointer");
     HFAGP_REQUIRE(a->B > 0 && a->H > 0 && a->W > 0, HFAGP_EBADARG, "torgb_skip: bad dims");
     HFAGP_REQUIRE(a->Cout % 32 == 0 && a->Cout <= 128 && a->Cin % CKB == 0 && a->Cin <= 512 && a->W % 32 == 0 &&
@@ -162,14 +179,21 @@
                   a->Cout, a->Cin, a->W, a->H * a->W);
     HFAGP_REQUIRE(!a->plane_major || a->Cout == 96, HFAGP_EUNSUPPORTED, "torgb_skip: plane_major needs Cout = 96 (3 planes x 32)");
     hipStream_t s = (hipStream_t)stream;
+    style_absmax = guard_table(style_absmax, a->styles);
     switch (kind_of(a->precision)) {
-        case 1: return launch_torgb_skip_kind<1>(a, s);
-        case 2: return launch_torgb_skip_kind<2>(a, s);
-        case 3: return launch_torgb_skip_kind<3>(a, s);
-        case 4: return launch_torgb_skip_kind<4>(a, s);
-        case 5: return launch_torgb_skip_kind<4>(a, s);
+        case 1: return launch_torgb_skip_kind<1>(a, style_absmax, s);
+        case 2: return launch_torgb_skip_kind<2>(a, style_absmax, s);
+        case 3: return launch_torgb_skip_kind<3>(a, style_absmax, s);
+        case 4: return launch_torgb_skip_kind<4>(a, style_absmax, s);
+        case 5: return launch_torgb_skip_kind<4>(a, style_absmax, s);
         default: break;
     }
     set_error("torgb_skip: precision %d has no 16-bit weight image", a->precision);
     return HFAGP_EBADARG;
 }
+
+extern "C" int hfagp_torgb_skip_fwd(const HfagpTorgbSkipArgs* a, void* stream) { return torgb_skip_fwd(a, nullptr, stream); }
+
+extern "C" int hfagp_torgb_skip_guard_fwd(const HfagpTorgbSkipArgs* a, const float* style_absmax, void* stream) {
+    return torgb_skip_fwd(a, style_absmax, stream);
+}
diff --git a/hfa-gp_amd/generator.py b/hfa-gp_amd/generator.py
--- a/hfa-gp_amd/generator.py
+++ b/hfa-gp_amd/generator.py
@@ -444,8 +444,9 @@
             main = torch.cuda.current_stream(x.device) if side is not None else None
             if side is not None:
                 side.wait_stream(main)
-                for t in (x, styles):
-                    t.record_stream(side)
+                for t in (x, styles, getattr(styles, "absmax", None)):
+                    if t is not None:
+                        t.record_stream(side)
             with (torch.cuda.stream(side) if side is not None else contextlib.nullcontext()):
                 self._planes_absmax = ops.absmax_slots(1, x.device)[0] if last else None
                 if conv_clamp is None and x.shape[0] == batch and ops.torgb_skip_supported(x, wt, tr.weight.shape[0]):
diff --git a/hfa-gp_amd/ops.py b/hfa-gp_amd/ops.py
--- a/hfa-gp_amd/ops.py
+++ b/hfa-gp_amd/ops.py
@@ -210,7 +210,11 @@
 def styles_demod_batch(items):
     arr = (L.StyleArgs * len(items))()
     out = [_style_args(a, "styles_demod_batch", *item) for a, item in zip(arr, items)]
-    L.check(L.lib().hfagp_style_batch_fwd(arr, len(items), _stream()), "style_batch_fwd")
+    table = torch.empty(len(items), max(s.shape[0] for s, _ in out), device=out[0][0].device, dtype=torch.float32)
+    rows = (C.c_void_p * len(items))(*[table[i].data_ptr() for i in range(len(items))])
+    L.check(L.lib().hfagp_style_batch_absmax_fwd(arr, rows, len(items), _stream()), "style_batch_absmax_fwd")
+    for i, (styles, _) in enumerate(out):
+        styles.absmax = table[i, :styles.shape[0]]
     return out
 
 
@@ -279,6 +283,13 @@
     L.check(L.lib().hfagp_fc_fwd(_ptr(x), _ptr(_chk(weight, "weight")), _ptr(bias), _ptr(y), b, fin, fout, lr_mul,
                                  _ACT[act], alpha, gain, _stream()), "fc_fwd")
     return y
+
+
+def _style_absmax(styles: Optional[torch.Tensor]) -> Optional[int]:
+    t = getattr(styles, "absmax", None) if styles is not None else None
+    if t is None or t.shape[0] != styles.shape[0] or t.device != styles.device:
+        return None
+    return t.data_ptr()
 
 
 def absmax_slots(n: int, device) -> torch.Tensor:
@@ -358,7 +369,7 @@
     if rgb_w is not None:
         part = torch.empty(L.lib().hfagp_modconv_rgb_parts(C.byref(a)), b, h, w, 4, device=x.device, dtype=torch.float32)
     a.workspace, a.rgb_part = _ptr(ws), _ptr(part)
-    L.check(L.lib().hfagp_modconv_fwd(C.byref(a), _stream()), "modconv_fwd")
+    L.check(L.lib().hfagp_modconv_guard_fwd(C.byref(a), _style_absmax(styles), _stream()), "modconv_fwd")
     return y if rgb_w is None else (y, part)
 
 
@@ -535,7 +546,7 @@
     a.img_out, a.x_absmax, a.out_absmax = _ptr(out), _ptr(x_absmax), _ptr(out_absmax)
     a.w_absmax = _ptr(getattr(wt, "w_absmax", None))
     a.B, a.H, a.W, a.Cin, a.Cout, a.plane_major = b, h, w, cin, cout, int(plane_major)
-    L.check(L.lib().hfagp_torgb_skip_fwd(C.byref(a), _stream()), "torgb_skip_fwd")
+    L.check(L.lib().hfagp_torgb_skip_guard_fwd(C.byref(a), _style_absmax(styles), _stream()), "torgb_skip_fwd")
     return out
 
 
diff --git a/include/hfagp.h b/include/hfagp.h
--- a/include/hfagp.h
+++ b/include/hfagp.h
@@ -143,6 +143,7 @@
 
 int hfagp_style_fwd(const HfagpStyleArgs* a, void* stream);
 int hfagp_style_batch_fwd(const HfagpStyleArgs* items, int32_t n, void* stream);
+int hfagp_style_batch_absmax_fwd(const HfagpStyleArgs* items, float* const* style_absmax, int32_t n, void* stream);
 
 int hfagp_qr_gram_fwd(const float* gram, const float* top, float* R, float* Rinv, int32_t n, void* stream);
 int hfagp_qr_refine_fwd(const float* gram, float* R, float* Rinv, float* status, int32_t n, void* stream);
@@ -214,6 +215,7 @@
 
 size_t hfagp_modconv_workspace_bytes(const HfagpModconvArgs* a);
 int hfagp_modconv_fwd(const HfagpModconvArgs* a, void* stream);
+int hfagp_modconv_guard_fwd(const HfagpModconvArgs* a, const float* style_absmax, void* stream);
 
 typedef struct {
     const void*  yt;
@@ -260,6 +262,7 @@
 } HfagpTorgbSkipArgs;
 
 int hfagp_torgb_skip_fwd(const HfagpTorgbSkipArgs* a, void* stream);
+int hfagp_torgb_skip_guard_fwd(const HfagpTorgbSkipArgs* a, const float* style_absmax, void* stream);
 
 typedef struct {
     const float* x;
```

Result: no change. 1038 frames/s, median of 6 (+0.8%).
